# rogerbarton/optix-renderer

Measured on AMD Instinct MI355X. Metric: Msamples/sec (whole node) + traversal HBM GB/s, cbox 1024x1024 256spp, higher is better.
Workload: dtype f32; 1 GPU; Cornell box (diffuse-only) 1024x1024, 16400 spp, path_mis; config=c2, width=1024, height=1024, spp=16400, mode=wavefront, traversal=ordered, pools=2, gpu_max_hw_queues=8, parallelism=single GPU

## Files before the change

### include/nori_hip.h

```cpp
#ifndef NORI_HIP_H
#define NORI_HIP_H

#include <stddef.h>
#include <stdint.h>

#ifdef __cplusplus
extern "C" {
#endif

#define NH_OK 0
#define NH_ERR_INVALID 1
#define NH_ERR_IO 2
#define NH_ERR_DEVICE 3
#define NH_ERR_UNSUPPORTED 4
#define NH_ERR_STATE 5


enum { NH_SHAPE_MESH = 0, NH_SHAPE_SPHERE = 1 };
enum { NH_BSDF_DIFFUSE = 0, NH_BSDF_MIRROR = 1, NH_BSDF_DIELECTRIC = 2, NH_BSDF_MICROFACET = 3, NH_BSDF_DISNEY = 4 };
enum { NH_EMITTER_AREA = 0, NH_EMITTER_POINT = 1, NH_EMITTER_ENVMAP = 2, NH_EMITTER_SPOT = 3,
       NH_EMITTER_DIRECTIONAL = 4 };
enum { NH_INTEGRATOR_PATH_MIS = 0, NH_INTEGRATOR_PATH_MATS = 1, NH_INTEGRATOR_DIRECT_EMS = 2,
       NH_INTEGRATOR_DIRECT_MATS = 3, NH_INTEGRATOR_DIRECT_MIS = 4, NH_INTEGRATOR_DIRECT = 5,
       NH_INTEGRATOR_NORMALS = 6,
// ... 171 lines not shown
    float bbox_max[3];
} nh_bvh_node;

typedef struct nh_bvh_desc {
    uint32_t n_nodes;
    const nh_bvh_node *nodes;
    uint32_t n_indices;
    const uint32_t *indices;
    uint32_t n_shapes;
    const uint32_t *shape_offset;
    float bbox_min[3], bbox_max[3];
    uint32_t max_depth;
} nh_bvh_desc;


typedef struct nh_ray_soa {
    const float *ox, *oy, *oz;
    const float *dx, *dy, *dz;
    const float *mint, *maxt;
} nh_ray_soa;

typedef struct nh_hit_soa {
    uint8_t *hit;
    float *t, *u, *v;
    uint32_t *prim;
    uint32_t *shape;
} nh_hit_soa;


enum { NH_MODE_MEGAKERNEL = 0, NH_MODE_WAVEFRONT = 1 };
enum { NH_TRAVERSAL_REFERENCE = 0, NH_TRAVERSAL_ORDERED = 1, NH_TRAVERSAL_WIDE = 2 };

typedef struct nh_render_req {
    int32_t sample_begin;
    int32_t sample_end;
    uint64_t seed;
    int32_t n_blocks;
    const int32_t *blocks;
    int32_t mode;
    int32_t traversal;
    int32_t clear;
    int32_t collect_stats;
} nh_render_req;

#define NH_SMALL_TABLES_BYTES 4096

typedef struct nh_render_stats {
    double kernel_ms_path;
    double kernel_ms_splat;
    double kernel_ms_extend;
    double kernel_ms_shadow;
    double kernel_ms_shade;
    uint64_t launches_path, launches_splat, launches_extend, launches_shadow, launches_shade;
    uint64_t samples;
    uint64_t ray_queries;
    uint64_t nodes_visited;
    uint64_t boxes_tested;
    uint64_t prims_tested;
    uint64_t invalid_samples;
    uint64_t shadow_queries, shadow_nodes_visited, shadow_boxes_tested, shadow_prims_tested;
    uint64_t shade_state_bytes, extend_queue_bytes, shadow_queue_bytes, paths_shaded;
    double kernel_ms_tail;
    uint64_t launches_tail;
    uint64_t node_bytes;
    uint64_t tail_queries, tail_nodes_visited, tail_boxes_tested, tail_prims_tested;
    uint64_t tail_shadow_queries, tail_shadow_nodes_visited, tail_shadow_boxes_tested, tail_shadow_prims_tested;
    uint64_t lds_scene;
    uint64_t fused_bounce;
    uint64_t comm_inits;
    double kernel_ms_denoise;
    uint64_t launches_denoise;
    uint64_t tails_async;
    uint64_t pools_active;
    uint64_t trace_fused;
    uint64_t tail_cycles_body, tail_cycles_shadow, tail_cycles_closest, tail_cycles_head;
    uint64_t tail_bounces, tail_max_bounces;
    uint64_t tail_coop_cycles_body, tail_coop_cycles_shadow, tail_coop_cycles_closest, tail_coop_cycles_head;
    uint64_t tail_coop_bounces;
    uint64_t bounce_cycles_load, bounce_cycles_body, bounce_cycles_shadow, bounce_cycles_closest, bounce_cycles_head;
    uint64_t bounce_cycles_store, bounce_bounces;
    uint64_t bounce_traits;
    uint64_t primary_masks;
    uint64_t pair_kinds;
} nh_render_stats;

typedef struct nh_scene nh_scene;
typedef struct nh_bvh nh_bvh;
typedef struct nh_ctx nh_ctx;

int nh_scene_load_xml(const char *path, nh_scene **out);
int nh_scene_load_xml_index(const char *path, int32_t index, nh_scene **out);
int nh_scene_get_desc(const nh_scene *scene, nh_scene_desc *out);
int nh_scene_set_resolution(nh_scene *scene, int32_t width, int32_t height);
int nh_scene_set_sample_count(nh_scene *scene, int32_t spp);
int nh_scene_set_sampler(nh_scene *scene, int32_t type, int32_t initial_uniform);
int nh_scene_set_bsdf(nh_scene *scene, uint32_t shape, const nh_bsdf *bsdf);
uint32_t nh_scene_add_texture(nh_scene *scene, const nh_texture *tex, const float *texels);
int nh_scene_set_normal_map(nh_scene *scene, uint32_t shape, uint32_t texture);
int nh_scene_set_lens_draw_order(nh_scene *scene, int32_t order);
int nh_texture_decode(const uint8_t *rgba8, uint64_t n, int32_t srgb, float *out);
int nh_scene_set_integrator(nh_scene *scene, int32_t integrator);
typedef struct nh_photon_params {
    int32_t photon_count;
    float photon_radius;
} nh_photon_params;
int nh_scene_get_photon_params(const nh_scene *scene, nh_photon_params *out);
int nh_scene_set_photon_params(nh_scene *scene, const nh_photon_params *params);
typedef struct nh_av_params {
    float length;
} nh_av_params;
int nh_scene_get_av_params(const nh_scene *scene, nh_av_params *out);
int nh_scene_set_av_params(nh_scene *scene, const nh_av_params *params);
int nh_photon_tables(float *cos_theta, float *sin_theta, float *cos_phi, float *sin_phi, float *exp_table);
void nh_scene_free(nh_scene *scene);
const char *nh_host_last_error(void);
int nh_debug_transform(const char *request, float *out, int32_t cap);

int nh_bvh_build(const nh_scene_desc *scene, int32_t n_threads, nh_bvh **out);
int nh_bvh_get_desc(const nh_bvh *bvh, nh_bvh_desc *out);
void nh_bvh_free(nh_bvh *bvh);

int nh_primary_masks(const nh_camera *camera, const float *records, int32_t n_records, const int32_t *blocks,
                     int32_t n_blocks, uint64_t *masks, int32_t *built);
int32_t nh_primary_mask_pad(int32_t width, int32_t height);

int nh_pair_layout(const float *records, int32_t n_records, const int32_t *leaves, int32_t n_leaves, int32_t by_kind,
                   int32_t *slots, int32_t *leaf_pairs);

int nh_framebuffer_to_rgb(const float *rgbw, int32_t width, int32_t height, int32_t border, float *rgb);
int nh_write_pfm(const char *path, const float *rgb, int32_t width, int32_t height);
int nh_image_load_png(const char *path, uint8_t *rgba, size_t cap, int32_t *width, int32_t *height);
int nh_write_exr(const char *path, const float *rgb, int32_t width, int32_t height);
int nh_rgb_to_ldr(const float *rgb, int32_t width, int32_t height, uint8_t *rgb8);
int nh_write_png(const char *path, const float *rgb, int32_t width, int32_t height);

int nh_get_device_count(int *n);
int nh_create(int device, nh_ctx **out);
void nh_destroy(nh_ctx *ctx);
int nh_upload_scene(nh_ctx *ctx, const nh_scene_desc *scene);
int nh_upload_bvh(nh_ctx *ctx, const nh_bvh_desc *bvh);
int nh_trace_rays(nh_ctx *ctx, const nh_ray_soa *rays, int32_t n, int32_t any_hit, int32_t traversal, nh_hit_soa *out);
#define NH_ADAPTIVE_MAX_SAMPLES 133948
#define NH_ADAPTIVE_STAGING_BYTES ((size_t)4 << 30)
int nh_render(nh_ctx *ctx, const nh_render_req *req);
typedef struct nh_adaptive_stats {
    uint64_t total_samples;
    uint64_t passes;
    uint64_t max_passes;
    uint64_t n_blocks;
} nh_adaptive_stats;
int nh_get_adaptive_stats(nh_ctx *ctx, nh_adaptive_stats *out);
int nh_get_adaptive_variance(nh_ctx *ctx, float *out, size_t n_floats);
int nh_synchronize(nh_ctx *ctx);
int nh_get_framebuffer(nh_ctx *ctx, float *rgbw, size_t n_floats);
int nh_framebuffer_device_ptr(nh_ctx *ctx, void **dptr, size_t *n_floats);
int nh_get_stats(nh_ctx *ctx, nh_render_stats *out);
int nh_reset_stats(nh_ctx *ctx);
int nh_reduce_framebuffers(nh_ctx **ctxs, int32_t n, int32_t root);
int nh_denoise(nh_ctx *ctx, const nh_denoiser *params);
int nh_denoise_image(nh_ctx *ctx, float *rgbw, int32_t width, int32_t height, int32_t border,
                     const nh_denoiser *params);
enum { NH_BSDF_QUERY_EVAL = 0, NH_BSDF_QUERY_SAMPLE = 1 };
int nh_bsdf_query(nh_ctx *ctx, const nh_bsdf *bsdf, const float *albedo, int32_t mode, int32_t n, const float *wi,
                  const float *wo, const float *sample, float *wo_out, float *value, float *pdf, int32_t *measure);
enum { NH_EMITTER_QUERY_SAMPLE = 0, NH_EMITTER_QUERY_EVAL = 1, NH_EMITTER_QUERY_PDF = 2,
       NH_EMITTER_QUERY_SAMPLE_PHOTON = 3 };
#define NH_EMITTER_QUERY_SAMPLE_STRIDE 16
#define NH_EMITTER_QUERY_PHOTON_STRIDE 12
#define NH_EMITTER_QUERY_IN_STRIDE 9
int nh_emitter_query(nh_ctx *ctx, uint32_t emitter, int32_t mode, int32_t n, const float *ref, const float *sample,
                     float *out);
enum { NH_MEDIUM_QUERY_FREE_PATH = 0, NH_MEDIUM_QUERY_TRANSMITTANCE = 1, NH_MEDIUM_QUERY_PHASE_SAMPLE = 2,
       NH_MEDIUM_QUERY_PHASE_PDF = 3 };
int nh_medium_query(nh_ctx *ctx, uint32_t medium, int32_t mode, int32_t n, const float *in, float *out);


enum { NH_TEST_TTEST = 0, NH_TEST_CHI2TEST = 1 };
typedef struct nh_test_desc {
    int32_t type;
    float significance_level;
    int32_t sample_count;
    uint32_t n_angles;
    const float *angles;
    uint32_t n_references;
    const float *references;
    uint32_t n_scenes;
    uint32_t n_bsdfs;
    const nh_bsdf *bsdfs;
} nh_test_desc;
typedef struct nh_test nh_test;
int nh_test_load_xml(const char *path, nh_test **out);
int nh_test_get_desc(const nh_test *test, nh_test_desc *out);
void nh_test_free(nh_test *test);

int nh_students_t_test(double mean, double variance, double reference, int32_t n, double alpha, int32_t num_tests,
                       int32_t *accepted, double *p_value);

#define NH_RADIANCE_QUERY_MAX (1 << 24)
int nh_radiance_query(nh_ctx *ctx, uint64_t seed, int32_t n, const int32_t *pixel, const int32_t *sample,
                      const float *pixel_sample, float *rgb, float *jitter);
int nh_ttest_scene(nh_ctx *ctx, uint64_t seed, int64_t first, int32_t n, double *mean, double *variance,
                   float *luminance);
int nh_ttest_bsdf(nh_ctx *ctx, const nh_bsdf *bsdf, const float *albedo, float angle_deg, uint64_t first_draw,
                  int32_t n, double *mean, double *variance, float *luminance);
typedef struct nh_test_result {
    double mean, variance, reference, p_value;
    int32_t accepted;
    int32_t sample_count;
    float angle;
    int32_t pad;
// ... 31 lines not shown
```

### optix-renderer_amd/csrc/nh_ctx.h

```cpp
#pragma once
#include <hip/hip_runtime.h>
#include <rccl/rccl.h>

#include <algorithm>
#include <cstdint>
#include <deque>
#include <memory>
#include <string>
#include <vector>

#include "nh_internal.h"
#include "nori_hip.h"

constexpr int kRing = 4;
constexpr int kPools = 4;
constexpr int kTails = 3;
constexpr int kTailCap = 65536;
#ifndef NH_DEFAULT_POOLS
#define NH_DEFAULT_POOLS 2
#endif

struct WfJob {
    uint64_t seq;
    int s0, rounds;
// ... 66 lines not shown
    std::vector<int32_t> list_key;
    bool have_list = false;
    void release() {
        for (int *p : {pixel_list, pixel_map, block_ids, block_slot, color_slots}) (void)hipFree(p);
        *this = PixelList{};
    }
};

struct AdaptiveState {
    int n_blocks = 0, nbx = 0, nby = 0;
    int next_sample = -1;
    int4 *blocks = nullptr;
    int *block_rank = nullptr, *active_list = nullptr, *next = nullptr;
    AdBlock *state = nullptr;
    unsigned *counts = nullptr, *h_count = nullptr;
    int2 *pos = nullptr;
    float4 *rad = nullptr, *staging = nullptr;
    float2 *jit = nullptr;
    size_t slot_cap = 0;
    unsigned long long *stats = nullptr;
    std::vector<int4> h_blocks;
};

struct PhotonState {
    bool built = false;
    std::vector<void *> bufs;
    const float *tables = nullptr;
    std::vector<float> h_tables;
    float *pos = nullptr;
    uint2 *bytes = nullptr;
    uint32_t *path = nullptr;
    int *bounce = nullptr;
    nh_photon_stats stats{};
};

struct nh_ctx {
    uint64_t id = 0;
    std::shared_ptr<CommSet> comms;
    int device = 0;
    hipStream_t stream = nullptr;
    std::string err;
    std::vector<nh_shape> shapes;
    std::vector<float> V;
    std::vector<uint32_t> F;
    int width = 0, height = 0, border = 0, n_emitters = 0, integrator = 0;
    nh_filter filter{};
    nhd::DScene S{};
    nhd::DScene *d_scene = nullptr;
    nhd::Traversal tv{};
    std::vector<void *> scene_bufs, bvh_bufs;
    bool has_scene = false, has_bvh = false;
    int depth = 0;
    int depth_wide = 0;
    int wide_w = 4;
    int n_node_f4 = 0, n_leaves = 0, n_prim_f4 = 0;
    std::vector<uint32_t> bvh_indices, shape_offset;
    std::vector<int> shape_bsdf_type;
    std::vector<int> shape_bsdf_real;
    int n_bsdf_types = 0;
    bool disney = false;
    bool specular = false;
    bool textured = false;
    bool normal_mapped = false;
    bool diffuse_area = false;
    bool bsdfless = false, has_media = false;
    int sampler = 0, adaptive_initial_uniform = 0;
    AdaptiveState ad;
    PhotonState photon;
    bool av_set = false;
    AvLaunch av{};
    std::vector<void *> av_bufs;
    size_t av_cap = 0;
    int2 *av_spill = nullptr;
    int av_spill_depth = 0;
    std::vector<nhd::DShape> h_shapes;
    std::vector<nhd::DBsdf> h_bsdfs;
    std::vector<nhd::DEmitter> h_emitters;
    std::vector<float> h_area_cdf;
    int n_emit_faces = 0;
    float4 *small_image = nullptr;
    int small_tab[5] = {0, 0, 0, 0, 0};
    bool pair_kinds = false;
    float4 *small_image_ref = nullptr;
    nh_camera camera{};
    std::vector<float> h_prims;
    unsigned long long *pmask = nullptr;
    bool pmask_known = false;
    float *fb = nullptr;
    size_t fb_floats = 0;
    float *rec = nullptr;
    size_t rec_cap = 0;
    int *block_rank = nullptr;
    int nbx = 0, nby = 0;
    PixelList px;
    float4 *staging = nullptr;
    size_t staging_cap = 0;
    unsigned long long *counters = nullptr;
    nh_render_stats stats{};
    WfPool pools[kPools + kTails];
    std::deque<WfJob> jobs;
    uint64_t job_seq = 0, splat_seq = 0;
    hipEvent_t fb_ev = nullptr;
    bool fb_ev_set = false;
    uint64_t stats_comm_inits = 0;
};

inline void drop_primary_masks(nh_ctx *c) {
    (void)hipFree(c->pmask);
    c->pmask = nullptr;
    c->pmask_known = false;
}

#define NH_LAUNCH(c, fn) ((c)->disney ? nh_disney::nh::fn : nh::fn)

void pool_free(WfPool &p);
int pipeline_drain(nh_ctx *c);
int check_device(nh_ctx *c, const char *where);
int render_adaptive(nh_ctx *c, const nh_render_req *q);
void adaptive_release(nh_ctx *c);
void photon_release(nh_ctx *c, bool tables = false);
nhd::DDisney disney_record(const nh_bsdf &b);
void disney_set_record(nhd::DBsdf &o, const nhd::DDisney *rec);
int disney_upload(nh_ctx *c, std::vector<void *> &owner, const std::vector<nhd::DDisney> &recs,
                  const std::vector<float> &albedo, nhd::DDisney **out);

int query_bsdf_record(nh_ctx *c, std::vector<void *> &owner, const nh_bsdf *b, const float *albedo, nhd::DBsdf &o,
                      float alb[3]);

inline bool fail(nh_ctx *c, const std::string &m) {
    if (c) c->err = m;
    return false;
}

#define HIP_TRY(ctx, expr)                                                                               \
    do {                                                                                                 \
        hipError_t e_ = (expr);                                                                          \
        if (e_ != hipSuccess) {                                                                          \
            (ctx)->err = std::string(#expr) + ": " + hipGetErrorString(e_);                              \
            return NH_ERR_DEVICE;                                                                        \
        }                                                                                                \
    } while (0)

template <typename T>
int upload(nh_ctx *c, std::vector<void *> &owner, const T *src, size_t n, const T **dst) {
    void *p = nullptr;
    size_t bytes = (std::max<size_t>(n * sizeof(T), 16) + 15) / 16 * 16;
    HIP_TRY(c, hipMalloc(&p, bytes));
    owner.push_back(p);
    if (n) HIP_TRY(c, hipMemcpyAsync(p, src, n * sizeof(T), hipMemcpyHostToDevice, c->stream));
    *dst = reinterpret_cast<const T *>(p);
    return NH_OK;
}

inline void free_all(std::vector<void *> &v) {
    for (void *p : v) (void)hipFree(p);
    v.clear();
}
```

### optix-renderer_amd/csrc/nh_internal.h

```cpp
#pragma once
#include <hip/hip_runtime.h>
#include <stdint.h>

#include "nh_device.h"
#include "nh_traverse.h"
#include "nori_hip.h"

struct RayBatch {
    const float *ox, *oy, *oz, *dx, *dy, *dz, *mint, *maxt;
};
struct HitBatch {
    uint8_t *hit;
    float *t, *u, *v;
    int *k;
};
#ifndef NH_REC_STRIDE
#define NH_REC_STRIDE 3
#endif
constexpr int kRecFloats = NH_REC_STRIDE;

struct PathLaunch {
    int n_paths;
    int n_list;
    int s0;
// ... 67 lines not shown
constexpr int kStatTailCoopClk = 32;
constexpr int kStatBounceClk = 40;
__device__ __forceinline__ unsigned long long *stat_shard(unsigned long long *c) {
    return c + (blockIdx.x & (kStatShards - 1)) * kStatStride;
}
__device__ __forceinline__ void flush_stats(const nhd::TravStats &st, uint32_t queries, unsigned long long *counters) {
    unsigned long long v[4] = {queries, st.nodes, st.boxes, st.prims};
#pragma unroll
    for (int i = 0; i < 4; ++i) {
        unsigned long long x = v[i];
#pragma unroll
        for (int off = 32; off > 0; off >>= 1) x += __shfl_xor(x, off, 64);
        if ((threadIdx.x & 63) == 0) atomicAdd(&counters[i], x);
    }
}

namespace nh {
void launch_trace(const nhd::DScene *S, const nhd::Traversal &tv, const RayBatch &rb, const HitBatch &hb, int n,
                  bool any, bool ordered, bool stats, int depth, unsigned long long *ctr, hipStream_t st);
void launch_trace_wide(const nhd::DScene *S, const nhd::Traversal &tv, const RayBatch &rb, const HitBatch &hb, int n,
                       bool any, bool ordered, bool stats, int2 *spill, int spill_depth, unsigned long long *ctr,
                       hipStream_t st, int wide = 4);
void launch_path(const nhd::DScene *S, const nhd::Traversal &tv, const PathLaunch &L, bool ordered, bool stats,
                 int depth, bool pm, hipStream_t st);
void launch_splat(const SplatLaunch &P, hipStream_t st);
void launch_av_primary(const nhd::DScene *S, const AvLaunch &L, hipStream_t st);
void launch_av_shade(const nhd::DScene *S, const nhd::Traversal &tv, const AvLaunch &L, hipStream_t st);
void launch_av_resolve(const AvLaunch &L, int bound, hipStream_t st);
bool splat_uses_staging(int border, int reach);
void launch_count_invalid(const float *rec, size_t n, unsigned long long *out, hipStream_t st);
void launch_denoise_variance(const DenoiseLaunch &P, hipStream_t st);
int denoise_band_rows();
int denoise_max_chunk();
int tree_top_nodes();
size_t denoise_tile_static_lds();
void launch_denoise_band(const DenoiseLaunch &P, int L, int n_bands, size_t tile_bytes, hipStream_t st);
void launch_denoise_copy(const float4 *src, int src_stride, float4 *dst, int dst_stride, int width, int height,
                         hipStream_t st);
}

constexpr int kQueueShards = 8, kCountStride = 32;

struct WfBuf {
    float4 *ray_o;
    float4 *ray_d;
    float4 *hit;
    uint64_t *rng;
    float4 *li;
    float4 *thr;
    float4 *pend;
    uint8_t *occl;
};
struct WfState {
    WfBuf buf[2];
    float4 *sh_o, *sh_d;
    int *sh_slot;
    unsigned *counts;
};
constexpr int kCountGroup = kQueueShards * kCountStride;
constexpr int kCountSlot = 4 * kCountGroup;

struct WfLaunch {
    WfState st;
    int n_paths, n_list, s0;
    uint64_t seed;
    const int *pixel_list;
    float *rec;
    float2 *jit;
    int in_q;
    int first;
    int cam_rays;
    unsigned *cnt_in;
    unsigned *cnt_out;
    int seg_cap;
    int small_nodes, small_leaves, small_prims;
    int small_frames;
    const float4 *small_image;
    int small_tab[5];
    uint32_t *trav_spill;
    int spill_depth;
    unsigned long long *counters;
    const unsigned long long *pmask;
    int pmask_nbx;
};
constexpr int kPersistentBlocks = 256 * 16;
constexpr size_t kSmallSceneBytes = 16384;
constexpr int kSmallFramesMaxPrims = 256;
constexpr size_t kSmallTablesBytes = NH_SMALL_TABLES_BYTES;
namespace nh {
void launch_wf_trace(const nhd::DScene *S, const nhd::Traversal &tv, const WfLaunch &L, bool ordered, bool stats,
                     bool shadow, bool persistent, int wide, int bound, int depth, hipStream_t st);
void launch_wf_trace2(const nhd::DScene *S, const nhd::Traversal &tv, const WfLaunch &L, bool ordered, bool stats,
                      int wide, int bound, hipStream_t st);
void launch_wf_camera_rays(const nhd::DScene *S, const WfLaunch &L, int bound, hipStream_t st);
void launch_wf_shade(const nhd::DScene *S, const nhd::Traversal &tv, const WfLaunch &L, bool sort, bool nmap, int bound,
                     hipStream_t st);
void launch_wf_bounce(const nhd::DScene *S, const nhd::Traversal &tv, const WfLaunch &L, bool ordered, bool stats,
                      bool sort, int bound, hipStream_t st);
void launch_wf_bounce_rr(const nhd::DScene *S, const nhd::Traversal &tv, const WfLaunch &L, bool ordered, bool stats, bool sort,
                         bool lean, bool nmap, bool trait, int bound, hipStream_t st);
void launch_wf_tail_rr(const nhd::DScene *S, const nhd::Traversal &tv, const WfLaunch &L, bool ordered, bool stats, int bound,
                       bool specular, bool lean, bool nmap, bool trait, hipStream_t st);
void launch_wf_bounce_trait(const nhd::DScene *S, const nhd::Traversal &tv, const WfLaunch &L, bool stats, int bound,
                            hipStream_t st);
void launch_wf_tail_trait(const nhd::DScene *S, const nhd::Traversal &tv, const WfLaunch &L, bool stats, int bound,
                          int coop, hipStream_t st);
void launch_wf_tail(const nhd::DScene *S, const nhd::Traversal &tv, const WfLaunch &L, bool ordered, bool stats,
                    int wide, int bound, int depth, hipStream_t st);
void launch_wf_pack_rr(const WfLaunch &L, const WfBuf &dst, unsigned *dst_counts, int bound, hipStream_t st);
void launch_small_image(const nhd::Traversal &tv, int n_prim_f4, const int2 *slots, int pairs_off, int frames_off,
                        float4 *image, hipStream_t st);
void launch_wf_counts(const unsigned *src, unsigned *host_dst, int n_copy, unsigned *zero, int n_zero, hipStream_t st);
}

namespace nh_disney {
namespace nh {
void launch_path(const nhd::DScene *S, const nhd::Traversal &tv, const PathLaunch &L, bool ordered, bool stats,
                 int depth, bool pm, hipStream_t st);
void launch_wf_shade(const nhd::DScene *S, const nhd::Traversal &tv, const WfLaunch &L, bool sort, bool nmap, int bound,
                     hipStream_t st);
void launch_wf_bounce(const nhd::DScene *S, const nhd::Traversal &tv, const WfLaunch &L, bool ordered, bool stats,
                      bool sort, int bound, hipStream_t st);
void launch_wf_bounce_rr(const nhd::DScene *S, const nhd::Traversal &tv, const WfLaunch &L, bool ordered, bool stats, bool sort,
                         bool lean, bool nmap, bool trait, int bound, hipStream_t st);
void launch_wf_tail_rr(const nhd::DScene *S, const nhd::Traversal &tv, const WfLaunch &L, bool ordered, bool stats, int bound,
                       bool specular, bool lean, bool nmap, bool trait, hipStream_t st);
void launch_wf_tail(const nhd::DScene *S, const nhd::Traversal &tv, const WfLaunch &L, bool ordered, bool stats,
                    int wide, int bound, int depth, hipStream_t st);
void launch_disney_fold(nhd::DDisney *recs, const float *albedo, int n, hipStream_t st);
struct BsdfQuery {
    nhd::DBsdf bsdf;
    float albedo[3];
    int mode, n;
    const float *wi, *wo, *sample;
    float *wo_out, *value, *pdf;
    int *measure;
};
void launch_bsdf_query(const BsdfQuery &q, hipStream_t st);
struct EmitterQuery {
    int emitter, mode, n;
    const float *ref, *in;
    float *out;
};
void launch_emitter_query(const nhd::DScene *S, const EmitterQuery &q, hipStream_t st);
void launch_vol_path(const nhd::DScene *S, const nhd::Traversal &tv, const PathLaunch &L, bool mis, bool stats, int depth,
                     hipStream_t st);
struct MediumQuery {
    int medium, mode, n;
    const float *in;
    float *out;
};
void launch_medium_query(const nhd::DScene *S, const MediumQuery &q, hipStream_t st);
}
}

struct PhotonTrace {
    uint64_t seed, k0;
    int n_paths;
    long long *counts;
    const long long *offsets;
    long long base;
    int cap;
    float *pos;
    uint2 *bytes;
    uint32_t *path;
    int *bounce;
// ... 110 lines not shown
```

### optix-renderer_amd/csrc/nh_layout.h

```cpp
#pragma once

namespace nhd {

constexpr int kLensLo = 256, kLensHi = 65536;

constexpr int kPrimSphere = 1, kPrimLeafEnd = 2, kPrimMatShift = 2;
constexpr int kPrimIsolated = 16;

constexpr int kWideF4 = 8;
constexpr int kWideEmpty = (int)0x80000000;

constexpr int kMaxStack = 128;

}
```

### optix-renderer_amd/csrc/nh_pipeline.hip

```cpp
#include <cmath>
#include <cstdlib>
#include <cstring>
#include <thread>
#include <type_traits>

#include "../host/gpu_layout.h"
#include "nh_ctx.h"


constexpr size_t kWfBytesPerPath = 2 * (16 * 6 + 8 + 1) + 36;

static int pool_alloc(nh_ctx *c, WfPool &p, size_t n, size_t rec_n, size_t staging_f4, bool jit = false) {
    if (!p.stream) {
        if (!p.h_counts && hipHostMalloc(reinterpret_cast<void **>(&p.h_counts),
                                         (kRing * 2 * kCountGroup + kCountSlot) * sizeof(unsigned)) != hipSuccess) {
            p.h_counts = nullptr;
            return fail(c, "hipHostMalloc failed"), NH_ERR_DEVICE;
        }
        for (hipEvent_t &e : p.copy_ev)
            if (!e) HIP_TRY(c, hipEventCreateWithFlags(&e, hipEventDisableTiming));
        for (hipEvent_t *e : {&p.ev_begin, &p.ev_path, &p.ev_splat0, &p.ev_splat})
            if (!*e) HIP_TRY(c, hipEventCreate(e));
        if (!p.ev_handoff) HIP_TRY(c, hipEventCreateWithFlags(&p.ev_handoff, hipEventDisableTiming));
        HIP_TRY(c, hipStreamCreateWithFlags(&p.stream, hipStreamNonBlocking));
// ... 112 lines not shown
}

static int pool_start(nh_ctx *c, WfPool &p, const WfJob &job) {
    WfJob j = job;
    j.staged = splat_staged(c);
    const char *jv = std::getenv("NH_SPLAT_JITTER");
    j.jit = jv && std::strcmp(jv, "stored") == 0;
    const int n_paths = j.rounds * c->px.n_list;
    const size_t staging_f4 = (size_t)j.rounds * c->px.n_blocks * block_px(c, j.staged);
    int rc = pool_alloc(c, p, (size_t)n_paths, (size_t)n_paths, staging_f4, j.jit);
    if (rc) return rc;
    for (int i = 0; i < active_pools(c); ++i) {
        WfPool &o = c->pools[i];
        if (&o == &p || o.state != WfPool::IDLE) continue;
        if ((rc = pool_alloc(c, o, (size_t)n_paths, (size_t)n_paths, staging_f4, j.jit))) return rc;
    }
    if (active_pools(c) > 1 && tail_async_enabled())
        for (int i = kPools; i < kPools + kTails; ++i) {
            WfPool &o = c->pools[i];
            if (o.state != WfPool::IDLE) continue;
            if ((rc = pool_alloc(c, o, (size_t)kTailCap, (size_t)n_paths, staging_f4, j.jit))) return rc;
        }
    p.job = j;
    WfLaunch &L = p.L;
    L = WfLaunch{};
    L.st = p.wf;
    L.n_paths = n_paths;
    L.n_list = c->px.n_list;
    L.s0 = j.s0;
    L.seed = j.seed;
    L.pixel_list = c->px.pixel_list;
    L.rec = p.rec;
    L.jit = j.jit ? p.jit : nullptr;
    L.counters = c->counters;
    const size_t scene_bytes = 16 * (size_t)(c->n_node_f4 + c->n_prim_f4) + 8 * (size_t)c->n_leaves;
    bool small = scene_bytes <= kSmallSceneBytes;
    if (const char *e = std::getenv("NH_LDS_SCENE")) small = small && e[0] != '0';
    if (small) {
        L.small_nodes = c->n_node_f4;
        L.small_leaves = c->n_leaves;
        L.small_prims = c->n_prim_f4;
        L.small_frames = c->n_prim_f4 / 3 <= kSmallFramesMaxPrims;
        if (const char *e = std::getenv("NH_LDS_FRAMES")) L.small_frames = L.small_frames && e[0] != '0';
        L.small_image = j.stats && c->small_image_ref ? c->small_image_ref : c->small_image;
        for (int i = 0; i < 5; ++i) L.small_tab[i] = c->small_tab[i];
    }
    const int per_chunk = 256;
    const int max_chunks = (n_paths + per_chunk - 1) / per_chunk;
    L.seg_cap = (max_chunks + kQueueShards - 1) / kQueueShards * per_chunk;
    p.persistent = c->depth > 20;
    if (const char *e = std::getenv("NH_PERSISTENT")) p.persistent = e[0] == '1';
    p.wide = p.persistent && j.ordered && c->tv.wnodes != nullptr;
    if (const char *e = std::getenv("NH_WIDE")) p.wide = p.wide && e[0] != '0';
    if (p.wide && !j.ordered) return fail(c, "wavefront pool: the wide traversal needs an ordered job"), NH_ERR_STATE;
    p.trace2 = p.wide && scene_bytes <= (size_t)256 << 20;
    if (const char *e = std::getenv("NH_TRACE2")) p.trace2 = p.wide && e[0] != '0';
    c->stats.trace_fused = p.trace2 ? 1 : 0;
    const int spill_words = p.wide ? 2 * c->depth_wide : (c->depth + 1) / 2 * 2;
    if (p.persistent && p.spill_words < spill_words) {
        HIP_TRY(c, hipStreamSynchronize(p.stream));
        (void)hipFree(p.spill);
        p.spill = nullptr;
        p.spill_words = 0;
        HIP_TRY(c, hipMalloc(&p.spill, (size_t)kPersistentBlocks * 128 * spill_words * sizeof(uint32_t)));
        p.spill_words = spill_words;
    }
    p.fused = small && !p.persistent && c->depth <= 16;
    if (const char *e = std::getenv("NH_FUSED")) p.fused = p.fused && e[0] != '0';
    p.sorted = p.fused && c->n_bsdf_types > 1;
    p.rr = p.fused;
    if (const char *e = std::getenv("NH_RR_AHEAD")) p.rr = p.fused && e[0] != '0';
    p.shade_sorted = false;
    if (const char *e = std::getenv("NH_SORT_SHADE")) p.shade_sorted = !p.fused && e[0] == '1';
    if (const char *e = std::getenv("NH_SORT")) p.sorted = p.fused && e[0] == '1';
    p.trait = p.rr && c->diffuse_area && c->small_tab[0] > 0 && j.ordered && !p.sorted;
    if (const char *e = std::getenv("NH_BOUNCE_TRAITS")) p.trait = p.trait && e[0] != '0';
    c->stats.bounce_traits = p.rr ? (p.trait ? 2 : 1) : 0;
    const char *pm = std::getenv("NH_PRIMARY_MASKS");
    const bool masks = p.rr && c->pmask && !j.stats && !(pm && pm[0] == '0');
    L.pmask = masks ? c->pmask : nullptr;
    L.pmask_nbx = c->nbx;
    c->stats.primary_masks = masks ? 1 : 0;
    c->stats.pair_kinds = p.fused && c->pair_kinds && !j.stats ? 1 : 0;
    c->stats.fused_bounce = p.fused ? 1 : 0;
    c->stats.node_bytes = p.wide ? 16 * nhd::kWideF4 * (c->wide_w / 4) : 64;
    c->stats.lds_scene = small && !p.persistent && c->depth <= 16 ? 1 : 0;
    L.trav_spill = p.spill;
    L.spill_depth = p.spill_words;
    p.tail_at = p.fused ? std::min<int64_t>(std::max<int64_t>(n_paths / 1024, 8192), 16384)
                        : std::min<int64_t>(std::max<int64_t>(n_paths / 64, 8192), 262144);
    if (const char *e = std::getenv("NH_TAIL")) p.tail_at = std::atoll(e);
    p.drain_at = std::max<int64_t>(n_paths / 8, p.tail_at);
    HIP_TRY(c, hipEventRecord(p.ev_begin, p.stream));
    unsigned *h_init = p.h_counts + kRing * 2 * kCountGroup;
    std::memset(h_init, 0, kCountSlot * sizeof(unsigned));
    h_init[0] = (unsigned)n_paths;
    HIP_TRY(c, hipMemcpyAsync(p.wf.counts, h_init, kCountSlot * sizeof(unsigned), hipMemcpyHostToDevice, p.stream));
    p.in_e.assign(1, (uint64_t)n_paths);
    p.in_s.assign(1, 0);
    p.it = 0;
    p.tail = false;
    p.draining = false;
    p.state = WfPool::ENQUEUE;
    return NH_OK;
}

static void chunk_swap(WfPool &a, WfPool &b) {
    std::swap(a.h_counts, b.h_counts);
    std::swap(a.copy_ev, b.copy_ev);
    std::swap(a.events, b.events);
    std::swap(a.ev_begin, b.ev_begin);
    std::swap(a.ev_path, b.ev_path);
    std::swap(a.ev_splat0, b.ev_splat0);
    std::swap(a.ev_splat, b.ev_splat);
    std::swap(a.job, b.job);
    std::swap(a.L, b.L);
    std::swap(a.persistent, b.persistent);
    std::swap(a.wide, b.wide);
    std::swap(a.trace2, b.trace2);
    std::swap(a.tail, b.tail);
    std::swap(a.draining, b.draining);
    std::swap(a.fused, b.fused);
    std::swap(a.sorted, b.sorted);
    std::swap(a.rr, b.rr);
    std::swap(a.trait, b.trait);
    std::swap(a.shade_sorted, b.shade_sorted);
    std::swap(a.tail_at, b.tail_at);
    std::swap(a.drain_at, b.drain_at);
    std::swap(a.it, b.it);
    std::swap(a.in_e, b.in_e);
    std::swap(a.in_s, b.in_s);
    std::swap(a.rec, b.rec);
    std::swap(a.rec_cap, b.rec_cap);
    std::swap(a.jit, b.jit);
    std::swap(a.jit_cap, b.jit_cap);
    std::swap(a.staging, b.staging);
    std::swap(a.staging_cap, b.staging_cap);
}

static WfPool *free_tail_slot(nh_ctx *c, const WfPool &p, int bound) {
    if (!p.rr || bound > kTailCap || active_pools(c) < 2) return nullptr;
    if (!tail_async_enabled()) return nullptr;
    for (int i = kPools; i < kPools + kTails; ++i)
        if (c->pools[i].state == WfPool::IDLE) return &c->pools[i];
    return nullptr;
}

static int pool_handoff(nh_ctx *c, WfPool &p, WfPool &T, int bound, hipEvent_t *ev) {
    int rc = pool_alloc(c, T, (size_t)kTailCap, 0, 0);
    if (rc) return rc;
    HIP_TRY(c, hipMemsetAsync(T.wf.counts, 0, kCountSlot * sizeof(unsigned), p.stream));
    nh::launch_wf_pack_rr(p.L, T.wf.buf[0], T.wf.counts, bound, p.stream);
    HIP_TRY(c, hipGetLastError());
    HIP_TRY(c, hipEventRecord(p.ev_handoff, p.stream));
    chunk_swap(p, T);
    WfLaunch &L = T.L;
    L.st = T.wf;
    L.in_q = 0;
    L.cnt_in = T.wf.counts;
    HIP_TRY(c, hipStreamWaitEvent(T.stream, p.ev_handoff, 0));
    HIP_TRY(c, hipEventRecord(ev[1], T.stream));
    HIP_TRY(c, hipEventRecord(ev[2], T.stream));
    NH_LAUNCH(c, launch_wf_tail_rr)(c->d_scene, c->tv, L, T.job.ordered, T.job.stats, bound, c->specular,
                          !c->specular && !c->textured, c->normal_mapped, T.trait, T.stream);
    HIP_TRY(c, hipGetLastError());
    HIP_TRY(c, hipEventRecord(ev[3], T.stream));
// ... 433 lines not shown
    c->av_cap = paths;
    c->av_spill_depth = spill_depth;
    return NH_OK;
}

static int av_chunk(nh_ctx *c, const nh_render_req *q, const PathLaunch &P) {
    AvLaunch L = c->av;
    L.n_paths = P.n_paths;
    L.n_list = P.n_list;
    L.s0 = P.s0;
    L.seed = P.seed;
    L.pixel_list = P.pixel_list;
    L.rec = P.rec;
    const bool wide = av_wide(c, q), ordered = q->traversal != NH_TRAVERSAL_REFERENCE, stats = q->collect_stats != 0;
    const auto batch = [&](float *const r[8], const HitBatch &hb, int n, bool any) {
        const RayBatch rb{r[0], r[1], r[2], r[3], r[4], r[5], r[6], r[7]};
        unsigned long long *ctr = c->counters + (any ? kStatAny : 0);
        if (wide) nh::launch_trace_wide(c->d_scene, c->tv, rb, hb, n, any, true, stats, c->av_spill, c->av_spill_depth, ctr,
                                        c->stream, c->wide_w);
        else nh::launch_trace(c->d_scene, c->tv, rb, hb, n, any, ordered, stats, c->depth, ctr, c->stream);
    };
    HIP_TRY(c, hipMemsetAsync(L.q_count, 0, sizeof(unsigned), c->stream));
    nh::launch_av_primary(c->d_scene, L, c->stream);
    batch(L.ray, L.hit, L.n_paths, false);
    nh::launch_av_shade(c->d_scene, c->tv, L, c->stream);
    HIP_TRY(c, hipGetLastError());
    int n_queue = L.n_paths;
    if (stats) {
        unsigned n = 0;
        HIP_TRY(c, hipMemcpyAsync(&n, L.q_count, sizeof(n), hipMemcpyDeviceToHost, c->stream));
        HIP_TRY(c, hipStreamSynchronize(c->stream));
        n_queue = (int)n;
    }
    HitBatch occl{};
    occl.hit = L.q_hit;
    batch(L.q_ray, occl, n_queue, true);
    nh::launch_av_resolve(L, n_queue, c->stream);
    return NH_OK;
}

extern "C" {

int nh_render(nh_ctx *c, const nh_render_req *q) {
    if (!c || !q) return NH_ERR_INVALID;
    if (!c->has_scene || !c->has_bvh) return fail(c, "nh_render: scene and BVH must be uploaded"), NH_ERR_STATE;
    if (q->sample_end < q->sample_begin || q->sample_begin < 0) return fail(c, "invalid sample range"), NH_ERR_INVALID;
    if (c->S.dof && q->sample_end > nhd::kLensLo * nhd::kLensHi)
        return fail(c, "depth of field: sample rounds beyond 2^24"), NH_ERR_UNSUPPORTED;
    if ((c->integrator == NH_INTEGRATOR_PATH_MIS || c->integrator == NH_INTEGRATOR_DIRECT_MIS) && c->n_emitters == 0)
        return fail(c, "No Emitter in scene!"), NH_ERR_INVALID;
    if (q->mode != NH_MODE_MEGAKERNEL && q->mode != NH_MODE_WAVEFRONT) return fail(c, "unknown render mode"), NH_ERR_INVALID;
    const bool volumetric = c->integrator == NH_INTEGRATOR_PATH_VOL_MATS || c->integrator == NH_INTEGRATOR_PATH_VOL_MIS;
    if (!volumetric && (c->bsdfless || c->has_media))
        return fail(c, "the scene has a participating medium or a shape without a BSDF: only the path_vol_mats and "
                       "path_vol_mis integrators render it"), NH_ERR_UNSUPPORTED;
    if (c->integrator == NH_INTEGRATOR_PATH_VOL_MIS && c->n_emitters == 0)
        return fail(c, "No Emitter in scene!"), NH_ERR_INVALID;
    const bool photon = c->integrator == NH_INTEGRATOR_PHOTONMAPPER;
    if (photon && !c->photon.built)
        return fail(c, "nh_render: the photon mapper needs a photon map (nh_photon_map_build)"), NH_ERR_STATE;
    if (photon && c->sampler == NH_SAMPLER_ADAPTIVE)
        return fail(c, "photonmapper: the adaptive sampler is not supported"), NH_ERR_UNSUPPORTED;
    if (c->integrator == NH_INTEGRATOR_AV && !c->av_set)
        return fail(c, "nh_render: the av integrator needs its length (nh_set_av_params)"), NH_ERR_STATE;
    if (c->integrator == NH_INTEGRATOR_ENVMAPTESTER && c->S.envmap < 0)
        return fail(c, "This integrator requires an env map."), NH_ERR_INVALID;
    const bool av_split = q->mode == NH_MODE_WAVEFRONT && c->integrator == NH_INTEGRATOR_AV;
    const bool wavefront = q->mode == NH_MODE_WAVEFRONT && c->integrator <= NH_INTEGRATOR_PATH_MATS;
    if (q->traversal < NH_TRAVERSAL_REFERENCE || q->traversal > NH_TRAVERSAL_WIDE)
        return fail(c, "unknown traversal"), NH_ERR_INVALID;
    if (c->border > 4) return fail(c, "reconstruction filters wider than border 4 are not supported"), NH_ERR_UNSUPPORTED;
    HIP_TRY(c, hipSetDevice(c->device));
    int rc = NH_OK;
    if (!wavefront || q->collect_stats || q->clear || c->sampler == NH_SAMPLER_ADAPTIVE) rc = pipeline_drain(c);
    if (rc) return rc;
    if (c->sampler == NH_SAMPLER_ADAPTIVE) return render_adaptive(c, q);
    rc = ensure_pixel_list(c, q);
    if (rc) return rc;
    if (wavefront && (rc = ensure_primary_masks(c))) return rc;
    c->stats.node_bytes = 64;
    if (av_split && av_wide(c, q)) c->stats.node_bytes = 16 * nhd::kWideF4 * (c->wide_w / 4);
    c->stats.primary_masks = 0;
    c->stats.pair_kinds = 0;
    c->stats.trace_fused = 0;
    c->stats.lds_scene = 0;
    c->stats.fused_bounce = 0;
    if (q->clear) {
        HIP_TRY(c, hipMemsetAsync(c->fb, 0, c->fb_floats * sizeof(float), c->stream));
        HIP_TRY(c, hipEventRecord(c->fb_ev, c->stream));
        c->fb_ev_set = true;
    }
    const int rounds = q->sample_end - q->sample_begin;
    if (rounds == 0 || c->px.n_list == 0) return NH_OK;
    if (q->collect_stats)
        HIP_TRY(c, hipMemsetAsync(c->counters, 0, kStatShards * kStatStride * sizeof(unsigned long long), c->stream));
    const size_t per_round = (size_t)c->px.n_list;
    const char *jv = std::getenv("NH_SPLAT_JITTER");
    const size_t rec_bytes = kRecFloats * 4 + (wavefront && jv && std::strcmp(jv, "stored") == 0 ? 8 : 0);
    const size_t per_round_bytes = per_round * rec_bytes + (size_t)c->px.n_blocks * block_px(c, splat_staged(c)) * 16 +
                                   (wavefront ? per_round * kWfBytesPerPath : 0) +
                                   (av_split ? per_round * av_bytes_per_path(c, q) : 0);
    size_t budget = wavefront ? (size_t)24 << 30 : (size_t)1 << 30;
    if (const char *e = std::getenv(wavefront ? "NH_WF_BUDGET_MB" : "NH_RECORD_BUDGET_MB"))
        budget = (size_t)std::max(1L, std::atol(e)) << 20;
    if (wavefront) {
        size_t free_b = 0, total_b = 0;
        if (hipMemGetInfo(&free_b, &total_b) == hipSuccess) {
            size_t held = 0;
            for (const WfPool &p : c->pools)
                held += p.cap * kWfBytesPerPath + p.rec_cap * kRecFloats * 4 + p.jit_cap * 8 + p.staging_cap * sizeof(float4);
            const int shares = active_pools(c) + (active_pools(c) > 1 && tail_async_enabled() ? kTails : 0);
            const size_t avail = (size_t)((double)(free_b + held) * 0.85) / (size_t)shares;
            budget = std::min(budget, std::max(avail, per_round_bytes));
        }
    }
    int chunk = (int)std::max<size_t>(1, std::min<size_t>((size_t)rounds, budget / per_round_bytes));
    while ((size_t)chunk * per_round > (size_t)0x7fffffff) chunk = std::max(1, chunk / 2);
    if (wavefront) {
        if (per_round > ((size_t)1 << 26))
            return fail(c, "wavefront mode renders at most 2^26 pixels per context"), NH_ERR_UNSUPPORTED;
        chunk = std::min(chunk, (int)(((size_t)1 << 26) / per_round));
    }

    if (wavefront) {
        HIP_TRY(c, hipStreamSynchronize(c->stream));
        for (int s = q->sample_begin; s < q->sample_end; s += chunk)
            c->jobs.push_back(WfJob{c->job_seq++, s, std::min(chunk, q->sample_end - s), q->seed,
                                    q->traversal != NH_TRAVERSAL_REFERENCE, q->collect_stats != 0});
        rc = q->collect_stats ? pipeline_drain(c) : pipeline_run(c, false);
        if (rc) return rc;
        if (int e = check_device(c, "nh_render")) return e;
    } else {
        if (c->rec_cap < (size_t)chunk * per_round) {
            (void)hipFree(c->rec);
            c->rec = nullptr;
            c->rec_cap = 0;
            const size_t cap = (size_t)chunk * per_round;
            HIP_TRY(c, hipMalloc(&c->rec, cap * kRecFloats * sizeof(float)));
            c->rec_cap = cap;
        }
        if (av_split && (rc = av_reserve(c, (size_t)chunk * per_round, av_wide(c, q)))) return rc;
        const bool staged = splat_staged(c);
        if (c->staging_cap < (size_t)chunk * c->px.n_blocks * block_px(c, staged)) {
            (void)hipFree(c->staging);
            c->staging = nullptr;
            c->staging_cap = 0;
            const size_t cap = (size_t)chunk * c->px.n_blocks * block_px(c, staged);
            HIP_TRY(c, hipMalloc(&c->staging, cap * sizeof(float4)));
            c->staging_cap = cap;
        }
        struct Ev {
            hipEvent_t a, b, d;
        };
        std::vector<Ev> evs;
        for (int s = q->sample_begin; s < q->sample_end; s += chunk) {
            const int k = std::min(chunk, q->sample_end - s);
            PathLaunch L{};
            L.n_paths = k * c->px.n_list;
            L.n_list = c->px.n_list;
            L.s0 = s;
            L.seed = q->seed;
            L.pixel_list = c->px.pixel_list;
            L.rec = c->rec;
            L.counters = c->counters;
            Ev ev;
            HIP_TRY(c, hipEventCreate(&ev.a));
// ... 86 lines not shown
```

### optix-renderer_amd/csrc/nh_traverse.h

```cpp
#pragma once
#include "nh_device.h"

namespace nhd {

struct Hit {
    float t, u, v;
    int k;
};

struct TravStats {
    uint32_t nodes, boxes, prims;
};

NHD bool box_test(float mnx, float mny, float mnz, float mxx, float mxy, float mxz, F3 o, F3 d, F3 r, float mint,
                  float maxt, float &near_out) {
    float near_t = -INFINITY, far_t = INFINITY;
    if (d.x == 0) {
        if (o.x < mnx || o.x > mxx) return false;
    } else {
        float t1 = (mnx - o.x) * r.x, t2 = (mxx - o.x) * r.x;
        if (t1 > t2) { float tmp = t1; t1 = t2; t2 = tmp; }
        near_t = e_max(t1, near_t);
        far_t = e_min(t2, far_t);
        if (!(near_t <= far_t)) return false;
    }
    if (d.y == 0) {
        if (o.y < mny || o.y > mxy) return false;
    } else {
        float t1 = (mny - o.y) * r.y, t2 = (mxy - o.y) * r.y;
        if (t1 > t2) { float tmp = t1; t1 = t2; t2 = tmp; }
        near_t = e_max(t1, near_t);
        far_t = e_min(t2, far_t);
        if (!(near_t <= far_t)) return false;
    }
    if (d.z == 0) {
        if (o.z < mnz || o.z > mxz) return false;
    } else {
        float t1 = (mnz - o.z) * r.z, t2 = (mxz - o.z) * r.z;
        if (t1 > t2) { float tmp = t1; t1 = t2; t2 = tmp; }
        near_t = e_max(t1, near_t);
        far_t = e_min(t2, far_t);
        if (!(near_t <= far_t)) return false;
    }
    near_out = near_t;
    return mint <= far_t && near_t <= maxt;
}

NHD float rcp_rn(float x) {
    const float r = __builtin_amdgcn_rcpf(x);
    const float e = __builtin_fmaf(-x, r, 1.0f);
    return __builtin_fmaf(e, r, r);
}
NHD float tri_inv_det(float det) {
    float r = rcp_rn(det);
    if (__builtin_expect(fabsf(det) >= 0x1p126f, 0)) r = 1.0f / det;
    return r;
}
NHD float dir_rcp(float x) {
    const float a = fabsf(x);
    if (__builtin_expect(a >= 0x1p-125f && a < 0x1p126f, 1)) return rcp_rn(x);
    return 1.0f / x;
}

NHD bool tri_test(float4 a, float4 b, float4 c, F3 o, F3 d, float mint, float maxt, float &t, float &u, float &v) {
    const F3 p0 = f3(a.x, a.y, a.z), e1 = sub(f3(b.x, b.y, b.z), p0), e2 = sub(f3(c.x, c.y, c.z), p0);
    F3 pvec = cross(d, e2);
    float det = dot(e1, pvec);
    if (det > -1e-8f && det < 1e-8f) return false;
    float inv_det = tri_inv_det(det);
    F3 tvec = sub(o, p0);
    u = dot(tvec, pvec) * inv_det;
    if (u < 0.0f || u > 1.0f) return false;
    F3 qvec = cross(tvec, e1);
    v = dot(d, qvec) * inv_det;
    if (v < 0.0f || u + v > 1.0f) return false;
    t = dot(e2, qvec) * inv_det;
    return t >= mint && t <= maxt;
}

typedef float f2 __attribute__((ext_vector_type(2)));
struct P3 {
    f2 x, y, z;
};
NHD P3 psub(P3 a, P3 b) { return P3{a.x - b.x, a.y - b.y, a.z - b.z}; }
// ... 49 lines not shown
    const float ax = (mnx - o.x) * r.x, bx = (mxx - o.x) * r.x;
    const float ay = (mny - o.y) * r.y, by = (mxy - o.y) * r.y;
    const float az = (mnz - o.z) * r.z, bz = (mxz - o.z) * r.z;
    const float near_t = fmaxf(fmaxf(fminf(ax, bx), fminf(ay, by)), fminf(az, bz));
    const float far_t = fminf(fminf(fmaxf(ax, bx), fmaxf(ay, by)), fmaxf(az, bz));
    near_out = near_t;
    return (near_t <= far_t) & (mint <= far_t) & (near_t <= maxt);
}

NHD void box_test_finite_pair(f2 mnx, f2 mny, f2 mnz, f2 mxx, f2 mxy, f2 mxz, float o_x, float o_y, float o_z,
                              float r_x, float r_y, float r_z, float mint, float maxt, bool &hit0, bool &hit1,
                              float &near0, float &near1) {
    const f2 ox{o_x, o_x}, oy{o_y, o_y}, oz{o_z, o_z}, rx{r_x, r_x}, ry{r_y, r_y}, rz{r_z, r_z};
    const f2 ax = (mnx - ox) * rx, bx = (mxx - ox) * rx;
    const f2 ay = (mny - oy) * ry, by = (mxy - oy) * ry;
    const f2 az = (mnz - oz) * rz, bz = (mxz - oz) * rz;
    const float n0 = fmaxf(fmaxf(fminf(ax.x, bx.x), fminf(ay.x, by.x)), fminf(az.x, bz.x));
    const float f0 = fminf(fminf(fmaxf(ax.x, bx.x), fmaxf(ay.x, by.x)), fmaxf(az.x, bz.x));
    const float n1 = fmaxf(fmaxf(fminf(ax.y, bx.y), fminf(ay.y, by.y)), fminf(az.y, bz.y));
    const float f1 = fminf(fminf(fmaxf(ax.y, bx.y), fmaxf(ay.y, by.y)), fmaxf(az.y, bz.y));
    near0 = n0;
    near1 = n1;
    hit0 = (n0 <= f0) & (mint <= f0) & (n0 <= maxt);
    hit1 = (n1 <= f1) & (mint <= f1) & (n1 <= maxt);
}

NHD bool sphere_test(float4 a, F3 o, F3 d, float mint, float maxt, float &t) {
    F3 L = sub(o, f3(a.x, a.y, a.z));
    float qa = dot(d, d);
    float qb = 2.f * dot(d, L);
    float qc = dot(L, L) - a.w * a.w;
    float discr = qb * qb - 4.f * qa * qc;
    if (discr < 0.f) return false;
    const float tmin = (-qb - f_sqrt(discr)) / 2 / qa;
    const float tmax = (-qb + f_sqrt(discr)) / 2 / qa;
    if (mint <= tmin && maxt >= tmin) { t = tmin; return true; }
    if (mint <= tmax && maxt >= tmax) { t = tmax; return true; }
    return false;
}

NHD void sphere_test_pair(f2 cx, f2 cy, f2 cz, f2 rad, F3 o, F3 d, f2 &tmin, f2 &tmax, bool &ok0, bool &ok1) {
    const P3 po{f2{o.x, o.x}, f2{o.y, o.y}, f2{o.z, o.z}}, pd{f2{d.x, d.x}, f2{d.y, d.y}, f2{d.z, d.z}};
    const P3 L = psub(po, P3{cx, cy, cz});
    const float qa = dot(d, d);
    const f2 qb = 2.f * pdot(pd, L);
    const f2 qc = pdot(L, L) - rad * rad;
    const f2 discr = qb * qb - (4.f * qa) * qc;
    ok0 = !(discr.x < 0.f);
    ok1 = !(discr.y < 0.f);
    tmin = tmax = f2{0.f, 0.f};
    if (ok0 | ok1) {
        const f2 s{f_sqrt(discr.x), f_sqrt(discr.y)};
        const f2 lo = (-qb - s) / 2, hi = (-qb + s) / 2;
        tmin = f2{lo.x / qa, lo.y / qa};
        tmax = f2{hi.x / qa, hi.y / qa};
    }
}
NHD bool sphere_in_range(float tmin, float tmax, float mint, float maxt, float &t) {
    const bool near_ok = mint <= tmin && maxt >= tmin;
    t = near_ok ? tmin : tmax;
    return near_ok || (mint <= tmax && maxt >= tmax);
}

NHD void accept_hit(bool hit, float t, float u, float v, int k, float &maxt, Hit &best, bool &found) {
    const bool up = hit && (t < maxt || k > best.k);
    maxt = up ? t : maxt;
    best.t = up ? t : best.t;
    best.u = up ? u : best.u;
    best.v = up ? v : best.v;
    best.k = up ? k : best.k;
    found = found || up;
}

struct Traversal {
    const float4 *nodes;
    const int2 *leaves;
    const float4 *prims;
    const float4 *wnodes;
    const float4 *ppairs;
    const int2 *pleaves;
    const float4 *frames;
    int n_top;
};
constexpr int kPairF4 = 6;

NHD bool prim_is_tri(float4 c) { return (__float_as_int(c.w) & kPrimSphere) == 0; }
NHD int prim_material(float4 c) { return (__float_as_int(c.w) >> kPrimMatShift) & 3; }

template <bool ANY, bool STATS, bool PAIRS = false, bool MASKED = false>
NHD bool leaf_test(const Traversal &tv, int leaf, F3 o, F3 d, float mint, float &maxt, Hit &best, bool &found,
                   TravStats &st, unsigned long long cand = ~0ull) {
    if constexpr (PAIRS && !STATS) {
        const int2 pl = tv.pleaves[leaf];
        if (pl.y) {
            const float4 *pp = tv.ppairs + (size_t)kPairF4 * pl.x;
            for (int i = 0, n = pl.y & 0xffff; i < n; ++i, pp += kPairF4) {
                const float4 q5 = pp[5];
                const int k0 = __float_as_int(q5.z), k1 = __float_as_int(q5.w);
                if constexpr (MASKED)
                    if (!(((cand >> (k0 & 63)) | (cand >> (k1 & 63))) & 1ull)) continue;
                const float4 q0 = pp[0], q1 = pp[1], q2 = pp[2], q3 = pp[3], q4 = pp[4];
                const P3 p0{f2{q0.x, q0.y}, f2{q0.z, q0.w}, f2{q1.x, q1.y}};
                const P3 e1{f2{q2.x, q2.y}, f2{q2.z, q2.w}, f2{q3.x, q3.y}};
                const P3 e2{f2{q3.z, q3.w}, f2{q4.x, q4.y}, f2{q4.z, q4.w}};
                f2 pt, pu, pv;
                bool ok0, ok1;
                tri_test_pair_e(p0, e1, e2, o, d, mint, pt, pu, pv, ok0, ok1);
                if (ANY) {
                    if ((ok0 && pt.x <= maxt) || (ok1 && pt.y <= maxt)) return true;
                    continue;
                }
                accept_hit(ok0 && pt.x <= maxt, pt.x, pu.x, pv.x, k0, maxt, best, found);
                accept_hit(ok1 && pt.y <= maxt, pt.y, pu.y, pv.y, k1, maxt, best, found);
            }
            for (int i = 0, n = pl.y >> 16; i < n; ++i, pp += kPairF4) {
                const float4 q5 = pp[5];
                const int k0 = __float_as_int(q5.z), k1 = __float_as_int(q5.w);
                if constexpr (MASKED)
                    if (!(((cand >> (k0 & 63)) | (cand >> (k1 & 63))) & 1ull)) continue;
                const float4 q0 = pp[0], q1 = pp[1];
                f2 tmin, tmax;
                bool ok0, ok1;
                sphere_test_pair(f2{q0.x, q0.y}, f2{q0.z, q0.w}, f2{q1.x, q1.y}, f2{q1.z, q1.w}, o, d, tmin, tmax, ok0, ok1);
                if (!(ok0 | ok1)) continue;
                float t0, t1;
                if (ANY) {
                    if ((sphere_in_range(tmin.x, tmax.x, mint, maxt, t0) && ok0) ||
                        (sphere_in_range(tmin.y, tmax.y, mint, maxt, t1) && ok1))
                        return true;
                    continue;
                }
                const bool h0 = sphere_in_range(tmin.x, tmax.x, mint, maxt, t0) && ok0;
                accept_hit(h0, t0, 0.f, 0.f, k0, maxt, best, found);
                const bool h1 = sphere_in_range(tmin.y, tmax.y, mint, maxt, t1) && ok1;
                accept_hit(h1, t1, 0.f, 0.f, k1, maxt, best, found);
            }
            return false;
        }
    }
    const int2 lf = tv.leaves[leaf];
    if constexpr (PAIRS) {
        for (int k = lf.x, e = lf.x + lf.y; k < e; k += 2) {
            if constexpr (MASKED && !STATS)
                if (!((cand >> (k & 63)) & 3ull)) continue;
            const float4 *pp = tv.ppairs + (size_t)kPairF4 * k;
            const float4 q0 = pp[0], q1 = pp[1], q2 = pp[2], q3 = pp[3], q4 = pp[4], q5 = pp[5];
            const P3 p0{f2{q0.x, q0.y}, f2{q0.z, q0.w}, f2{q1.x, q1.y}};
            const P3 e1{f2{q2.x, q2.y}, f2{q2.z, q2.w}, f2{q3.x, q3.y}};
            const P3 e2{f2{q3.z, q3.w}, f2{q4.x, q4.y}, f2{q4.z, q4.w}};
            f2 pt, pu, pv;
            bool ok0, ok1;
            tri_test_pair_e(p0, e1, e2, o, d, mint, pt, pu, pv, ok0, ok1);
            const bool has1 = k + 1 < e;
            if (!STATS && !((__float_as_int(q5.x) | (has1 ? __float_as_int(q5.y) : 0)) & kPrimSphere)) {
                if (ANY) {
                    if ((ok0 && pt.x <= maxt) || (has1 && ok1 && pt.y <= maxt)) return true;
                    continue;
                }
                const bool h0 = ok0 && pt.x <= maxt;
                const bool u0 = h0 && (pt.x < maxt || k > best.k);
                maxt = u0 ? pt.x : maxt;
                best.t = u0 ? pt.x : best.t;
                best.u = u0 ? pu.x : best.u;
                best.v = u0 ? pv.x : best.v;
                best.k = u0 ? k : best.k;
                const bool h1 = has1 && ok1 && pt.y <= maxt;
                const bool u1 = h1 && (pt.y < maxt || k + 1 > best.k);
// ... 141 lines not shown
    if (fin) {
        box_test_finite_pair(f2{l0, r0}, f2{l1, r1}, f2{l2, r2}, f2{l3, r3}, f2{l4, r4}, f2{l5, r5}, o.x, o.y, o.z, r.x,
                             r.y, r.z, mint, maxt, hl, hr, nl, nr);
    } else {
        hl = box_test(l0, l1, l2, l3, l4, l5, o, d, r, mint, maxt, nl);
        hr = box_test(r0, r1, r2, r3, r4, r5, o, d, r, mint, maxt, nr);
    }
}

template <int DEPTH, bool ORDERED, bool ANY, bool STATS, bool PAIRS = false, int G = 1, bool RCP = false,
          bool MASKED = false>
NHD bool trace(const Traversal &tv, const DScene &S, F3 o, F3 d, float mint, float maxt, Hit &best, uint32_t *stk,
               int stride, TravStats &st, unsigned long long cand = ~0ull) {
    if (mint == kEps) mint = e_max(mint, mint * e_max(fabsf(o.x), e_max(fabsf(o.y), fabsf(o.z))));
    const bool lead = G == 1 || (threadIdx.x & (G - 1)) == 0;
    best.k = -1;
    best.t = INFINITY;
    if (S.root_kind == 0 || maxt < mint) return false;
    const F3 r = RCP ? f3(dir_rcp(d.x), dir_rcp(d.y), dir_rcp(d.z)) : f3(1.0f / d.x, 1.0f / d.y, 1.0f / d.z);
    const bool fin = isfinite(r.x) & isfinite(r.y) & isfinite(r.z);
    bool found = false;
    float near_t;
    if (STATS && lead) st.boxes++;
    if (fin ? !box_test_finite(S.root_min[0], S.root_min[1], S.root_min[2], S.root_max[0], S.root_max[1],
                               S.root_max[2], o, r, mint, maxt, near_t)
            : !box_test(S.root_min[0], S.root_min[1], S.root_min[2], S.root_max[0], S.root_max[1], S.root_max[2], o,
                        d, r, mint, maxt, near_t))
        return false;
    if (S.root_kind == 2) {
        bool any = leaf_any<ANY, STATS, PAIRS, G, MASKED>(tv, 0, o, d, mint, maxt, best, found, st, cand);
        return ANY ? any : found;
    }
    int sp = 0;
    int cur = 0;
    for (;;) {
        while (cur >= 0) {
            const float *nf = node_f(tv, cur);
            const int ref_l = node_ref(nf, 0), ref_r = node_ref(nf, 1);
            if (STATS && lead) { st.nodes++; st.boxes += 2; }
            float nl, nr;
            bool hl, hr;
            node_box_tests(nf, o, d, r, mint, maxt, fin, hl, hr, nl, nr);
            int next;
            if (hl && hr) {
                const bool right_first = ORDERED && nr < nl;
                stk[sp * stride] = ((uint32_t)cur << 1) | (right_first ? 0u : 1u);
                ++sp;
                next = right_first ? ref_r : ref_l;
            } else if (hl) {
                next = ref_l;
            } else if (hr) {
                next = ref_r;
            } else {
                break;
            }
            if (next >= 0) {
                cur = next;
                continue;
            }
            if (leaf_any<ANY, STATS, PAIRS, G, MASKED>(tv, ~next, o, d, mint, maxt, best, found, st, cand)) return true;
            break;
        }
        cur = -1;
        while (sp > 0) {
            --sp;
            const uint32_t e = stk[sp * stride];
            const int parent = (int)(e >> 1), side = (int)(e & 1u);
            const float *nf = node_f(tv, parent);
            if (STATS && lead) st.boxes++;
            if (!child_box_test(nf, side, o, d, r, mint, maxt, near_t, fin)) continue;
            const int ref = node_ref(nf, side);
            if (ref >= 0) {
                cur = ref;
                break;
            }
            if (leaf_any<ANY, STATS, PAIRS, G, MASKED>(tv, ~ref, o, d, mint, maxt, best, found, st, cand)) return true;
        }
        if (cur < 0) break;
    }
    (void)DEPTH;
    return ANY ? false : found;
}

template <bool STATS, int G = 1>
NHD bool iso_sphere_hit(const Traversal &tv, int k_prev, F3 o, F3 d, float mint, float maxt, Hit &best,
                        TravStats &st) {
    if (k_prev < 0) return false;
    const float4 c = tv.prims[3 * k_prev + 2];
    if (!(__float_as_int(c.w) & kPrimIsolated)) return false;
    if (mint == kEps) mint = e_max(mint, mint * e_max(fabsf(o.x), e_max(fabsf(o.y), fabsf(o.z))));
    if (maxt < mint) return false;
    const float4 a = tv.prims[3 * k_prev];
    const float lim = a.w + tv.prims[3 * k_prev + 1].x;
    if (!(fabsf(o.x - a.x) <= lim && fabsf(o.y - a.y) <= lim && fabsf(o.z - a.z) <= lim)) return false;
    float t;
    if (!sphere_test(a, o, d, mint, maxt, t) || !(t >= 2.f * mint)) return false;
    best.t = t;
    best.u = 0.f;
    best.v = 0.f;
    best.k = k_prev;
    if (STATS && (G == 1 || (threadIdx.x & (G - 1)) == 0)) st.prims++;
    return true;
}

template <int DEPTH, bool ORDERED, bool STATS, bool PAIRS = false, int G = 1, bool ISO = true, bool RCP = false>
NHD bool trace_next(const Traversal &tv, const DScene &S, int k_prev, F3 o, F3 d, float mint, float maxt, Hit &best,
                    uint32_t *stk, int stride, TravStats &st) {
#ifndef NH_AB_NO_ISO
    if (ISO && S.iso_spheres && S.root_kind != 0 && iso_sphere_hit<STATS, G>(tv, k_prev, o, d, mint, maxt, best, st))
        return true;
#endif
    return trace<DEPTH, ORDERED, false, STATS, PAIRS, G, RCP>(tv, S, o, d, mint, maxt, best, stk, stride, st);
}



template <int K>
struct RingStack {
    static_assert((K & (K - 1)) == 0, "K must be a power of two");
    uint32_t *lds;
    int stride;
    uint32_t *glob;
    NHD void push(int i, uint32_t e) {
        uint32_t *slot = lds + (i & (K - 1)) * stride;
        if (i >= K) glob[i - K] = *slot;
        *slot = e;
    }
    NHD uint32_t pop(int i) {
        uint32_t *slot = lds + (i & (K - 1)) * stride;
        const uint32_t e = *slot;
        if (i >= K) *slot = glob[i - K];
        return e;
    }
};

template <bool ORDERED, bool ANY, bool STATS, class Stack>
struct Tracer {
    F3 o, d, r;
    float mint, maxt;
    int cur;
    int k, kend;
    int sp;
    bool found, done;
    bool fin;
    Hit best;

    NHD void begin(const DScene &S, const Traversal &tv, F3 o_, F3 d_, float mint_, float maxt_, TravStats &st) {
        o = o_;
        d = d_;
        mint = mint_;
        maxt = maxt_;
        if (mint == kEps) mint = e_max(mint, mint * e_max(fabsf(o.x), e_max(fabsf(o.y), fabsf(o.z))));
        best.k = -1;
        best.t = INFINITY;
        found = false;
        done = true;
        sp = 0;
        cur = -1;
        k = kend = 0;
        if (S.root_kind == 0 || maxt < mint) return;
        r = f3(1.0f / d.x, 1.0f / d.y, 1.0f / d.z);
        fin = isfinite(r.x) & isfinite(r.y) & isfinite(r.z);
        float near_t;
        if (STATS) st.boxes++;
        if (fin ? !box_test_finite(S.root_min[0], S.root_min[1], S.root_min[2], S.root_max[0], S.root_max[1],
                                   S.root_max[2], o, r, mint, maxt, near_t)
                : !box_test(S.root_min[0], S.root_min[1], S.root_min[2], S.root_max[0], S.root_max[1], S.root_max[2],
                            o, d, r, mint, maxt, near_t))
            return;
        done = false;
        if (S.root_kind == 2) {
            const int2 lf = tv.leaves[0];
            k = lf.x;
            kend = lf.x + lf.y;
        } else {
            cur = 0;
        }
    }

    NHD void step(const Traversal &tv, Stack &stk, TravStats &st) {
        if (k < kend) {
            const float4 a = tv.prims[3 * k], b = tv.prims[3 * k + 1], c = tv.prims[3 * k + 2];
            if (STATS) st.prims++;
            float t, u = 0.f, v = 0.f;
            const bool hit = prim_is_tri(c) ? tri_test(a, b, c, o, d, mint, maxt, t, u, v)
                                                        : sphere_test(a, o, d, mint, maxt, t);
            if (hit) {
                if (ANY) {
                    found = true;
                    done = true;
                    return;
                }
                if (t < maxt || k > best.k) {
                    found = true;
                    maxt = t;
// ... 486 lines not shown
```

### optix-renderer_amd/csrc/nh_upload.hip

```cpp
#include <cmath>
#include <cstdlib>
#include <cstring>

#include "../host/gpu_layout.h"
#include "nh_ctx.h"

using nhd::DBsdf;
using nhd::DEmitter;
using nhd::DShape;

static_assert(sizeof(nh::f4) == sizeof(float4) && alignof(float4) % alignof(nh::f4) == 0, "nh::f4 is float4's layout");
static_assert(sizeof(nh::i2) == sizeof(int2) && alignof(int2) % alignof(nh::i2) == 0, "nh::i2 is int2's layout");
static_assert(sizeof(nh::u64x2) == sizeof(ulonglong2) && alignof(ulonglong2) % alignof(nh::u64x2) == 0,
              "nh::u64x2 is ulonglong2's layout");
static_assert((int)nhd::BSDF_DIELECTRIC == (int)NH_BSDF_DIELECTRIC, "the isolated-sphere marking reads NH_BSDF_*");

nhd::DDisney disney_record(const nh_bsdf &b) {
    nhd::DDisney o;
    std::memset(&o, 0, sizeof(o));
    o.metallic = b.metallic; o.subsurface = b.subsurface; o.specular = b.specular; o.roughness = b.roughness;
    o.specular_tint = b.specular_tint; o.anisotropic = b.anisotropic; o.sheen = b.sheen; o.sheen_tint = b.sheen_tint;
    o.clearcoat = b.clearcoat; o.clearcoat_gloss = b.clearcoat_gloss;
    return o;
}
// ... 280 lines not shown
    for (int i = 0; i < 3; ++i) S.ndir[i] = d->normals_direction[i];
    std::memcpy(S.s2c, d->camera.sample_to_camera, sizeof(S.s2c));
    std::memcpy(S.c2w, d->camera.camera_to_world, sizeof(S.c2w));
    {
        float ow[4];
        const float z = 0.0f;
        for (int i = 0; i < 4; ++i) {
            float acc = S.c2w[4 * i] * z;
            acc = acc + S.c2w[4 * i + 1] * z;
            acc = acc + S.c2w[4 * i + 2] * z;
            acc = acc + S.c2w[4 * i + 3] * 1.0f;
            ow[i] = acc;
        }
        for (int i = 0; i < 3; ++i) S.cam_o[i] = ow[i] / ow[3];
    }
    S.inv_w = d->camera.inv_output_size[0];
    S.inv_h = d->camera.inv_output_size[1];
    S.near_clip = d->camera.near_clip;
    S.far_clip = d->camera.far_clip;
    S.width = d->camera.width;
    S.height = d->camera.height;
    S.dof = d->camera.lens_radius > 1e-4f ? 1 : 0;
    S.lens_radius = d->camera.lens_radius;
    S.focal_distance = d->camera.focal_distance;
    S.lens_rtl = d->camera.lens_draw_order == NH_LENS_DRAWS_RTL ? 1 : 0;
    S.lens_pix = S.lens_lo = nullptr;
    S.lens_hi = nullptr;
    if (S.dof) {
        const nh::LensTables lt = nh::lens_tables(S.width, S.height);
        const nh::u64x2 *pix = nullptr, *lo = nullptr;
        if ((rc = upload(c, c->scene_bufs, lt.pix.data(), lt.pix.size(), &pix))) return rc;
        if ((rc = upload(c, c->scene_bufs, lt.lo.data(), lt.lo.size(), &lo))) return rc;
        if ((rc = upload(c, c->scene_bufs, lt.hi.data(), lt.hi.size(), &S.lens_hi))) return rc;
        S.lens_pix = reinterpret_cast<const ulonglong2 *>(pix);
        S.lens_lo = reinterpret_cast<const ulonglong2 *>(lo);
        HIP_TRY(c, hipStreamSynchronize(c->stream));
    }
    S.filter_radius = d->filter.radius;
    S.lookup = d->filter.lookup_factor;
    S.border = d->filter.border;
    std::memcpy(S.table, d->filter.table, sizeof(S.table));

    c->shapes.assign(d->shapes, d->shapes + d->n_shapes);
    c->shape_bsdf_type.clear();
    c->shape_bsdf_real.clear();
    unsigned types = 0;
    for (uint32_t i = 0; i < d->n_shapes; ++i) {
        const int t = d->shapes[i].bsdf < 0 ? NH_BSDF_DIFFUSE : d->bsdfs[d->shapes[i].bsdf].type;
        c->shape_bsdf_real.push_back(t);
        types |= 1u << t;
    }
    int disney_key = 0;
    for (int k : {NH_BSDF_MICROFACET, NH_BSDF_MIRROR, NH_BSDF_DIELECTRIC, NH_BSDF_DIFFUSE})
        if (!(types & (1u << k))) {
            disney_key = k;
            break;
        }
    for (int t : c->shape_bsdf_real) c->shape_bsdf_type.push_back(t == NH_BSDF_DISNEY ? disney_key : t);
    c->disney = (types & (1u << NH_BSDF_DISNEY)) != 0;
    c->disney = c->disney || !dx.empty();
    c->n_bsdf_types = __builtin_popcount(types);
    c->specular = (types & ((1u << NH_BSDF_MIRROR) | (1u << NH_BSDF_DIELECTRIC))) != 0;
    c->textured = false;
    for (uint32_t i = 0; i < d->n_bsdfs; ++i) c->textured = c->textured || d->bsdfs[i].albedo_texture != 0;
    c->normal_mapped = false;
    for (uint32_t i = 0; i < d->n_shapes; ++i) c->normal_mapped = c->normal_mapped || d->shapes[i].normal_map != 0;
    c->textured = c->textured || c->normal_mapped;
    c->diffuse_area = S.integrator == NH_INTEGRATOR_PATH_MIS && !c->textured && !S.dof && d->envmap < 0 &&
                      d->n_emitters > 0;
    for (uint32_t i = 0; i < d->n_bsdfs; ++i) c->diffuse_area = c->diffuse_area && d->bsdfs[i].type == NH_BSDF_DIFFUSE;
    for (uint32_t i = 0; i < d->n_emitters; ++i) {
        const nh_emitter &e = d->emitters[i];
        c->diffuse_area = c->diffuse_area && e.type == NH_EMITTER_AREA && e.shape >= 0 &&
                          (uint32_t)e.shape < d->n_shapes && ds[e.shape].ef_off >= 0;
    }
    for (uint32_t i = 0; i < d->n_shapes; ++i)
        c->diffuse_area = c->diffuse_area && d->shapes[i].emitter < (int32_t)d->n_emitters;
    c->h_shapes = ds;
    c->h_bsdfs = db;
    c->h_emitters = de;
    c->h_area_cdf.assign(d->area_cdf, d->area_cdf + d->n_area_cdf);
    c->n_emit_faces = (int)ef_tri.size();
    c->small_image = c->small_image_ref = nullptr;
    c->pair_kinds = false;
    c->V.assign(d->V, d->V + 3 * nv);
    c->F.assign(d->F, d->F + 3 * (size_t)d->n_faces);
    c->width = d->camera.width;
    c->height = d->camera.height;
    c->border = d->filter.border;
    c->filter = d->filter;
    c->n_emitters = (int)d->n_emitters;
    c->integrator = S.integrator;
    if (d->sampler != NH_SAMPLER_INDEPENDENT && d->sampler != NH_SAMPLER_ADAPTIVE)
        return fail(c, "unknown sampler"), NH_ERR_INVALID;
    c->sampler = d->sampler;
    c->adaptive_initial_uniform = std::max(1, (int)d->adaptive_initial_uniform);
    adaptive_release(c);
    photon_release(c);
    c->av_set = false;

    (void)hipFree(c->fb);
    c->fb = nullptr;
    c->fb_floats = 4 * (size_t)(c->width + 2 * c->border) * (size_t)(c->height + 2 * c->border);
    HIP_TRY(c, hipMalloc(&c->fb, c->fb_floats * sizeof(float)));
    HIP_TRY(c, hipMemsetAsync(c->fb, 0, c->fb_floats * sizeof(float), c->stream));
    auto rank = nh::spiral_rank(c->width, c->height, 32, c->nbx, c->nby);
    (void)hipFree(c->block_rank);
    HIP_TRY(c, hipMalloc(&c->block_rank, rank.size() * sizeof(int)));
    HIP_TRY(c, hipMemcpyAsync(c->block_rank, rank.data(), rank.size() * sizeof(int), hipMemcpyHostToDevice, c->stream));
    HIP_TRY(c, hipStreamSynchronize(c->stream));
    c->has_scene = true;
    return NH_OK;
}

static int build_small_image(nh_ctx *c, const nh::GpuBvh &g) {
    c->small_image = c->small_image_ref = nullptr;
    c->pair_kinds = false;
    for (int &v : c->small_tab) v = 0;
    const size_t scene_bytes = 16 * (size_t)(c->n_node_f4 + c->n_prim_f4) + 8 * (size_t)c->n_leaves;
    if (scene_bytes > kSmallSceneBytes) return NH_OK;
    const int n = c->n_prim_f4 / 3;
    const int leaves_f4 = (c->n_leaves + 1) / 2;
    const int pairs_off = c->n_node_f4 + c->n_prim_f4 + leaves_f4;
    const bool frames = n <= kSmallFramesMaxPrims;
    std::vector<float4> tab;
    if (c->diffuse_area) {
        std::vector<nhd::DShape> sh = c->h_shapes;
        std::vector<float> cdf;
        for (const nhd::DEmitter &e : c->h_emitters) {
            nhd::DShape &s = sh[e.shape];
            if ((size_t)s.pdf_off + s.n_faces + 1 > c->h_area_cdf.size()) return fail(c, "area CDF out of range"), NH_ERR_INVALID;
            const int off = (int)cdf.size();
            cdf.insert(cdf.end(), c->h_area_cdf.begin() + s.pdf_off, c->h_area_cdf.begin() + s.pdf_off + s.n_faces + 1);
            s.pdf_off = off;
        }
        cdf.resize((cdf.size() + 3) / 4 * 4, 0.f);
        const size_t bytes = sh.size() * sizeof(nhd::DShape) + c->h_bsdfs.size() * sizeof(nhd::DBsdf) +
                             c->h_emitters.size() * sizeof(nhd::DEmitter) + cdf.size() * sizeof(float) +
                             3 * (size_t)c->n_emit_faces * sizeof(float4);
        if (bytes <= kSmallTablesBytes) {
            static_assert(sizeof(nhd::DShape) % 16 == 0 && sizeof(nhd::DBsdf) % 16 == 0 && sizeof(nhd::DEmitter) % 16 == 0,
                          "table records are whole float4s");
            c->small_tab[0] = (int)(sh.size() * sizeof(nhd::DShape) / 16);
            c->small_tab[1] = (int)(c->h_bsdfs.size() * sizeof(nhd::DBsdf) / 16);
            c->small_tab[2] = (int)(c->h_emitters.size() * sizeof(nhd::DEmitter) / 16);
            c->small_tab[3] = (int)(cdf.size() / 4);
            c->small_tab[4] = 3 * c->n_emit_faces;
            tab.resize((size_t)c->small_tab[0] + c->small_tab[1] + c->small_tab[2] + c->small_tab[3]);
            char *w = reinterpret_cast<char *>(tab.data());
            std::memcpy(w, sh.data(), sh.size() * sizeof(nhd::DShape));
            w += sh.size() * sizeof(nhd::DShape);
            std::memcpy(w, c->h_bsdfs.data(), c->h_bsdfs.size() * sizeof(nhd::DBsdf));
            w += c->h_bsdfs.size() * sizeof(nhd::DBsdf);
            std::memcpy(w, c->h_emitters.data(), c->h_emitters.size() * sizeof(nhd::DEmitter));
            w += c->h_emitters.size() * sizeof(nhd::DEmitter);
            std::memcpy(w, cdf.data(), cdf.size() * sizeof(float));
        }
    }
    const int tab_f4 = (int)tab.size() + c->small_tab[4];
    const int pleaves_off = pairs_off + nhd::kPairF4 * n, tab_off = pleaves_off + leaves_f4;
    const int frames_off = tab_off + tab_f4;
    const size_t total = (size_t)frames_off + (frames ? 3 * (size_t)n : 0);
    const auto d2d = [&](float4 *dst, const void *src, size_t bytes) {
        return bytes ? hipMemcpyAsync(dst, src, bytes, hipMemcpyDeviceToDevice, c->stream) : hipSuccess;
    };
    const char *pk = std::getenv("NH_PAIR_KINDS");
    c->pair_kinds = n > 0 && !(pk && pk[0] == '0');
    for (int pass = 0; pass < (c->pair_kinds ? 2 : 1); ++pass) {
        const bool by_kind = c->pair_kinds && pass == 0;
        const nh::PairLayout pl = nh::pair_layout(g.leaves.data(), c->n_leaves, g.prims.data(), n, by_kind);
        float4 *img = nullptr;
        HIP_TRY(c, hipMalloc(&img, std::max<size_t>(total, 1) * sizeof(float4)));
        c->bvh_bufs.push_back(img);
        HIP_TRY(c, hipMemsetAsync(img, 0, std::max<size_t>(total, 1) * sizeof(float4), c->stream));
        HIP_TRY(c, d2d(img, c->tv.nodes, 16 * (size_t)c->n_node_f4));
        HIP_TRY(c, d2d(img + c->n_node_f4, c->tv.prims, 16 * (size_t)c->n_prim_f4));
        HIP_TRY(c, d2d(img + c->n_node_f4 + c->n_prim_f4, c->tv.leaves, 8 * (size_t)c->n_leaves));
        if (n > 0) {
            const nh::i2 *slots = nullptr;
            if (int rc = upload(c, c->bvh_bufs, pl.slots.data(), pl.slots.size(), &slots)) return rc;
            nh::launch_small_image(c->tv, c->n_prim_f4, reinterpret_cast<const int2 *>(slots), pairs_off,
                                   frames ? frames_off : -1, img, c->stream);
            HIP_TRY(c, hipGetLastError());
        }
        if (c->n_leaves > 0)
            HIP_TRY(c, hipMemcpyAsync(img + pleaves_off, pl.leaves.data(), 8 * (size_t)c->n_leaves, hipMemcpyHostToDevice,
                                      c->stream));
        if (!tab.empty()) {
            float4 *t = img + tab_off;
            HIP_TRY(c, hipMemcpyAsync(t, tab.data(), tab.size() * sizeof(float4), hipMemcpyHostToDevice, c->stream));
            HIP_TRY(c, d2d(t + tab.size(), c->S.emit_faces, 16 * (size_t)c->small_tab[4]));
        }
        HIP_TRY(c, hipStreamSynchronize(c->stream));
        (pass == 0 ? c->small_image : c->small_image_ref) = img;
    }
    return NH_OK;
}

int nh_set_av_params(nh_ctx *c, const nh_av_params *params) {
    if (!c) return NH_ERR_INVALID;
    if (!params || std::isnan(params->length)) return fail(c, "nh_set_av_params: invalid av parameters"), NH_ERR_INVALID;
    if (!c->has_scene) return fail(c, "nh_set_av_params: no scene uploaded"), NH_ERR_STATE;
    HIP_TRY(c, hipSetDevice(c->device));
    if (int rc = pipeline_drain(c)) return rc;
    HIP_TRY(c, hipStreamSynchronize(c->stream));
    c->S.av_length = params->length;
    if (c->d_scene && c->has_bvh)
        HIP_TRY(c, hipMemcpy(reinterpret_cast<char *>(c->d_scene) + offsetof(nhd::DScene, av_length), &c->S.av_length,
                             sizeof(float), hipMemcpyHostToDevice));
    c->av_set = true;
    return NH_OK;
}

int nh_upload_bvh(nh_ctx *c, const nh_bvh_desc *b) {
    if (!c || !b) return NH_ERR_INVALID;
    if (!c->has_scene) return fail(c, "nh_upload_bvh: upload the scene first"), NH_ERR_STATE;
    HIP_TRY(c, hipSetDevice(c->device));
    if (int rc_ = pipeline_drain(c)) return rc_;
    HIP_TRY(c, hipStreamSynchronize(c->stream));
    free_all(c->bvh_bufs);
    c->has_bvh = false;
    photon_release(c);
    c->wide_w = std::getenv("NH_WIDE8") && std::getenv("NH_WIDE8")[0] == '1' ? 8 : 4;
    int top_k = nh::tree_top_nodes() * 4 / c->wide_w;
    if (const char *e = std::getenv("NH_TREE_TOP")) top_k = std::min(std::max(0, std::atoi(e)), top_k);
    nh::GpuBvh g;
    if (int rc_ = nh::build_gpu_bvh(*b, c->shapes, c->V, c->F, c->shape_bsdf_type, c->shape_bsdf_real, c->wide_w, top_k,
                                    g, c->err))
        return rc_;
    nhd::DScene &S = c->S;
    S.root_kind = g.root_kind;
    for (int i = 0; i < 3; ++i) { S.root_min[i] = g.root_min[i]; S.root_max[i] = g.root_max[i]; }
    S.iso_spheres = g.iso_spheres;
    c->tv.n_top = g.n_top;
    int rc;
    c->n_node_f4 = (int)g.nodes.size();
    c->n_leaves = (int)g.leaves.size();
    c->n_prim_f4 = (int)g.prims.size() - 3;
    drop_primary_masks(c);
    c->h_prims.clear();
    if (c->n_prim_f4 > 0 && c->n_prim_f4 / 3 <= 64)
        c->h_prims.assign(&g.prims[0].x, &g.prims[0].x + 4 * (size_t)c->n_prim_f4);
    const nh::f4 *nodes = nullptr, *prims = nullptr, *wide = nullptr;
    const nh::i2 *leaves = nullptr;
    if ((rc = upload(c, c->bvh_bufs, g.nodes.data(), g.nodes.size(), &nodes))) return rc;
    if ((rc = upload(c, c->bvh_bufs, g.leaves.data(), g.leaves.size(), &leaves))) return rc;
    if ((rc = upload(c, c->bvh_bufs, g.prims.data(), g.prims.size(), &prims))) return rc;
    if (!g.wide.empty() && (rc = upload(c, c->bvh_bufs, g.wide.data(), g.wide.size(), &wide))) return rc;
    c->tv.nodes = reinterpret_cast<const float4 *>(nodes);
    c->tv.leaves = reinterpret_cast<const int2 *>(leaves);
    c->tv.prims = reinterpret_cast<const float4 *>(prims);
    c->tv.wnodes = reinterpret_cast<const float4 *>(wide);
    c->depth_wide = g.depth_wide;
    S.nodes = c->tv.nodes;
    S.prims = c->tv.prims;
    c->bvh_indices.assign(b->indices, b->indices + b->n_indices);
    c->shape_offset = g.shape_offset;
    c->depth = (int)g.tree_depth + 2;
    if (!c->d_scene) HIP_TRY(c, hipMalloc(&c->d_scene, sizeof(nhd::DScene)));
    HIP_TRY(c, hipMemcpyAsync(c->d_scene, &c->S, sizeof(nhd::DScene), hipMemcpyHostToDevice, c->stream));
    if ((rc = build_small_image(c, g))) return rc;
    HIP_TRY(c, hipStreamSynchronize(c->stream));
    c->has_bvh = true;
    return NH_OK;
}

}
```

### optix-renderer_amd/csrc/nh_wavefront.hip

```cpp
#include "nh_dispatch.h"
#include "nh_internal.h"
#include "nh_shade.h"

#include <algorithm>
#include <cstdlib>

using namespace nhd;

#ifdef NH_DISNEY
namespace nh_disney {
#endif

namespace {

enum : int { F_DISCRETE = 1, F_NEE = 2, F_ZERO_COL = 4, F_ZNAN = 8, F_FIRST = 64 };
constexpr int kPidBits = 26;

__device__ __forceinline__ int wave_append(unsigned *counter, bool pred) {
    const unsigned long long mask = __ballot(pred);
    const int lane = threadIdx.x & 63;
    const int leader = __ffsll((long long)mask) - 1;
    unsigned base = 0;
    if (mask != 0ull && lane == leader) base = atomicAdd(counter, (unsigned)__popcll(mask));
    base = __shfl(base, leader < 0 ? 0 : leader, 64);
// ... 922 lines not shown
#pragma unroll
        for (int c = 0; c < kMatClasses; ++c) {
            const int r = wave_append(&s_n[c], cont && cls == c);
            if (cls == c) rank = r;
        }
    } else {
        cls = 0;
        rank = wave_append(&s_n[0], cont);
    }
    __syncthreads();
    if (threadIdx.x == 0) {
        unsigned tot = 0;
        for (int c = 0; c < kMatClasses; ++c) {
            s_off[c] = tot;
            tot += s_n[c];
        }
        s_base = tot ? atomicAdd(&L.cnt_out[shard * kCountStride], tot) : 0u;
    }
    __syncthreads();
    if (cont) {
        const WfBuf &Bo = L.st.buf[1 - L.in_q];
        const int slot = shard * L.seg_cap + (int)(s_base + s_off[cls]) + rank;
        store_state(Bo, slot, o);
        Bo.hit[slot] = hit_out;
    }
    if (STATS) {
        flush_trav_stats(stat_shard(L.counters), q_e, st_e);
        flush_trav_stats(stat_shard(L.counters) + kStatAny, q_s, st_s);
    }
}

__device__ __forceinline__ void store_post_head(const WfBuf &B, int s, const PathV &v, const Hit &h) {
    B.ray_o[s] = make_float4(v.org.x, v.org.y, v.org.z, 0.f);
    B.ray_d[s] = make_float4(v.d.x, v.d.y, v.d.z, __int_as_float((int)(((unsigned)(v.flags & 0x30) << kPidBits) | (unsigned)v.pid)));
    B.li[s] = make_float4(v.li.x, v.li.y, v.li.z, v.w_mats);
    B.thr[s] = make_float4(v.t.x, v.t.y, v.t.z, v.w_ems);
    B.rng[s] = v.rng.state;
    B.hit[s] = make_float4(h.t, h.u, h.v, __int_as_float(h.k));
}

struct RawState {
    float4 ro, rd, li4, th4, hv;
    uint64_t rng;
};
__device__ __forceinline__ RawState load_raw_state(const WfBuf &B, int s) {
    RawState r;
    r.ro = B.ray_o[s];
    r.rd = B.ray_d[s];
    r.li4 = B.li[s];
    r.th4 = B.thr[s];
    r.hv = B.hit[s];
    r.rng = B.rng[s];
    return r;
}

template <bool NMAP = true, class ST = DScene>
__device__ __forceinline__ void unpack_post_head(const DScene &S, const ST &T, const Traversal &tv, const WfLaunch &L,
                                                 const RawState &r, PathV &v, Hit &h, Its &its) {
    const float4 ro = r.ro, rd = r.rd, li4 = r.li4, th4 = r.th4, hv = r.hv;
    v.rng.state = r.rng;
    const int bits = __float_as_int(rd.w);
    v.flags = (int)((unsigned)bits >> kPidBits);
    v.pid = bits & ((1 << kPidBits) - 1);
    v.rng.inc = ((uint64_t)(L.s0 + v.pid / L.n_list) << 1u) | 1u;
    v.org = xyz(ro);
    v.d = xyz(rd);
    v.li = xyz(li4);
    v.w_mats = li4.w;
    v.t = xyz(th4);
    v.w_ems = th4.w;
    h.t = hv.x;
    h.u = hv.y;
    h.v = hv.z;
    h.k = __float_as_int(hv.w);
    hit_info<NMAP>(S, T.shapes, tv, h, v.org, v.d, its);
}

template <bool NMAP = true, class ST = DScene>
__device__ __forceinline__ void load_post_head(const DScene &S, const ST &T, const Traversal &tv, const WfLaunch &L,
                                               const WfBuf &B, int s, PathV &v, Hit &h, Its &its) {
    unpack_post_head<NMAP>(S, T, tv, L, load_raw_state(B, s), v, h, its);
}

template <bool ORDERED, bool STATS, bool NMAP = true, bool TRAIT = false, class ST = DScene>
__device__ __forceinline__ bool first_vertex(const DScene &S, const ST &T, const Traversal &tv, const WfLaunch &L, int s,
                                             PathV &v, Hit &h, Its &its, uint32_t *stk, int stride, TravStats &st_e,
                                             unsigned long long &q_e) {
    float4 ro, rd;
    float jx, jy;
#ifndef NH_AB_NO_PMASK
    constexpr bool MASKED = !STATS;
#else
    constexpr bool MASKED = false;
#endif
    unsigned long long cand = ~0ull;
    if constexpr (MASKED) {
        int blk;
        camera_sample<!TRAIT>(S, L, s, v.rng, ro, rd, jx, jy, &blk);
        if (L.pmask) cand = L.pmask[blk];
    } else {
        camera_sample<!TRAIT>(S, L, s, v.rng, ro, rd, jx, jy);
    }
    if (L.jit) L.jit[s] = make_float2(jx, jy);
    v.org = xyz(ro);
    v.d = xyz(rd);
    v.li = f3(0.f, 0.f, 0.f);
    v.t = f3(1.f, 1.f, 1.f);
    v.w_mats = 1.f;
    v.w_ems = 0.f;
    v.flags = F_FIRST;
    v.pid = s;
    const bool live = rd.w >= ro.w;
    q_e += live ? 1 : 0;
    const bool found =
        live && trace<16, ORDERED, false, STATS, true, 1, TRAIT, MASKED>(tv, S, v.org, v.d, ro.w, rd.w, h, stk, stride,
                                                                        st_e, cand);
    if (!shade_head<NMAP, TRAIT>(S, T, tv, v, h, found, 0.f, its)) {
        write_radiance(L, v);
        return false;
    }
    return true;
}

struct TailClocks {
    unsigned long long c[4] = {0, 0, 0, 0};
    unsigned long long bounces = 0, max_bounces = 0;
    unsigned long long cc[4] = {0, 0, 0, 0}, coop_bounces = 0;
};

template <bool ORDERED, bool STATS, bool CLK = false, int G = 1, bool FULL = true, bool NMAP = FULL, bool TRAIT = false,
          bool LEAN = false, class ST = DScene>
__device__ __forceinline__ bool rr_step(const DScene &S, const ST &T, const Traversal &tv, const WfLaunch &L, PathV &v, Its &its,
                                        Hit &h, uint32_t *stk, int stride, TravStats &st_e, TravStats &st_s,
                                        unsigned long long &q_e, unsigned long long &q_s, TailClocks *clk = nullptr) {
    const bool lead = G == 1 || (threadIdx.x & (G - 1)) == 0;
    PState o;
    bool nee = false;
    float4 so, sd;
    unsigned long long t0 = 0, t1 = 0;
    unsigned long long *cs = CLK ? (G > 1 ? clk->cc : clk->c) : nullptr;
    if constexpr (CLK) t0 = clock64();
    [[maybe_unused]] const uint64_t inc = v.rng.inc;
    shade_body<FULL, TRAIT>(S, T, tv, v, its, o, nee, so, sd);
    if constexpr (CLK) {
        t1 = clock64();
        if (lead) cs[0] += t1 - t0;
        t0 = t1;
    }
    if (nee) {
        Hit hs;
        if (lead) ++q_s;
        if (!trace<16, ORDERED, true, STATS, true, G, TRAIT>(tv, S, xyz(so), xyz(sd), so.w, sd.w, hs, stk, stride, st_s)) {
            o.li.x = o.li.x + o.pe.x;
            o.li.y = o.li.y + o.pe.y;
            o.li.z = o.li.z + o.pe.z;
            o.thr.w = o.pe.w;
        } else if (o.flags & F_ZNAN) {
            o.li.x = o.li.x + NAN;
            o.li.y = o.li.y + NAN;
            o.li.z = o.li.z + NAN;
        }
        o.flags &= ~(F_NEE | F_ZNAN);
    }
    if constexpr (CLK) {
        t1 = clock64();
        if (lead) cs[1] += t1 - t0;
        t0 = t1;
    }
    const bool live = o.rd.w >= o.ro.w;
    if (lead) q_e += live ? 1 : 0;
    const bool found = live && trace_next<16, ORDERED, STATS, true, G, FULL, TRAIT>(tv, S, h.k, xyz(o.ro), xyz(o.rd),
                                                                             o.ro.w, o.rd.w, h, stk, stride, st_e);
    if constexpr (CLK) {
        t1 = clock64();
        if (lead) cs[2] += t1 - t0;
        t0 = t1;
    }
    if constexpr (TRAIT) {
        v.org = xyz(o.ro);
        v.d = xyz(o.rd);
        v.li = xyz(o.li);
        v.w_mats = o.li.w;
        v.t = xyz(o.thr);
        v.w_ems = o.thr.w;
        v.rng.state = o.rng;
        v.rng.inc = inc;
        v.flags = o.flags;
        v.pid = o.pid;
    } else {
        v = path_of(L, o);
    }
    const bool alive = shade_head<NMAP, TRAIT, LEAN>(S, T, tv, v, h, found, o.pdfmat, its);
    if constexpr (CLK) {
        if (lead) cs[3] += clock64() - t0;
        if (lead) ++(G > 1 ? clk->coop_bounces : clk->bounces);
    }
    if (!alive) {
        if (lead) write_radiance(L, v);
        return false;
    }
    return true;
}

#ifndef NH_BOUNCE_TB
#define NH_BOUNCE_TB 256
#endif

template <bool ORDERED, bool STATS, bool FULL, bool NMAP = FULL, bool TRAIT = false, int BOUNCE = -1, class ST = DScene>
__device__ __forceinline__ bool bounce_path(const DScene &S, const ST &T, const Traversal &tv, const WfLaunch &L, const QView &qv,
                                            int q, uint32_t *my_stk, PathV &v, Hit &h, TravStats &st_e,
                                            TravStats &st_s, unsigned long long &q_e, unsigned long long &q_s,
                                            TailClocks &clk, unsigned long long &c_load, const RawState *pre = nullptr) {
    Its its;
    bool alive = true;
    unsigned long long t_ph = 0;
    if constexpr (STATS) t_ph = clock64();
    const bool first = BOUNCE < 0 ? L.first != 0 : BOUNCE == 0;
    if (first) {
        const int s = queue_slot(qv.pre, L.seg_cap, q);
        alive = first_vertex<ORDERED, STATS, NMAP, TRAIT>(S, T, tv, L, s, v, h, its, my_stk, NH_BOUNCE_TB, st_e, q_e);
    } else if (BOUNCE == 1) {
        unpack_post_head<NMAP>(S, T, tv, L, *pre, v, h, its);
    } else {
        load_post_head<NMAP>(S, T, tv, L, L.st.buf[L.in_q], queue_slot(qv.pre, L.seg_cap, q), v, h, its);
    }
    if constexpr (STATS) c_load += clock64() - t_ph;
    return alive && rr_step<ORDERED, STATS, STATS, 1, FULL, NMAP, TRAIT, true>(S, T, tv, L, v, its, h, my_stk,
                                                                         NH_BOUNCE_TB, st_e, st_s, q_e, q_s, &clk);
}

template <bool ORDERED, bool STATS, bool SORT, bool FULL = true, bool NMAP = FULL, bool TRAIT = false, int BOUNCE = -1>
__global__ __launch_bounds__(NH_BOUNCE_TB, NH_DZ_WAVES(true, NH_BOUNCE_WAVES)) void wf_bounce_rr(const DScene *__restrict__ Sp, Traversal tv_g,
                                                                     WfLaunch L) {
    __shared__ uint32_t stk[16 * NH_BOUNCE_TB];
    __shared__ unsigned s_n[kMatClasses], s_off[kMatClasses], s_base;
    extern __shared__ float4 lds_scene[];
    const QView qv = queue_view(L.cnt_in);
    const int base = blockIdx.x * NH_BOUNCE_TB;
    if (base >= qv.n) return;
    if (threadIdx.x < kMatClasses) s_n[threadIdx.x] = 0u;
    const DScene &S = *Sp;
    const int q = base + (int)threadIdx.x;
    [[maybe_unused]] RawState pre;
    if constexpr (BOUNCE == 1)
        if (q < qv.n) pre = load_raw_state(L.st.buf[L.in_q], queue_slot(qv.pre, L.seg_cap, q));
    const Traversal tv = stage_small_scene<true>(tv_g, L, lds_scene);
    const int shard = blockIdx.x & (kQueueShards - 1);
    uint32_t *my_stk = stk + threadIdx.x;
    TravStats st_e{0, 0, 0}, st_s{0, 0, 0};
    unsigned long long q_e = 0, q_s = 0;
    bool cont = false;
    PathV v;
    Hit h;
    int cls = kMatClasses - 1;
    TailClocks clk;
    unsigned long long c_load = 0, c_store = 0, t_ph = 0;
    if (q < qv.n) {
        const auto &T = scene_tables<TRAIT && NH_TRAIT_TABLES>(S, L, lds_scene);
        cont = bounce_path<ORDERED, STATS, FULL, NMAP, TRAIT, BOUNCE>(S, T, tv, L, qv, q, my_stk, v, h, st_e, st_s, q_e, q_s,
                                                                      clk, c_load, BOUNCE == 1 ? &pre : nullptr);
        if (cont) cls = prim_material(tv.prims[3 * h.k + 2]);
        if constexpr (STATS) t_ph = clock64();
    }
    int rank = 0;
    if (SORT) {
#pragma unroll
        for (int c = 0; c < kMatClasses; ++c) {
            const int r = wave_append(&s_n[c], cont && cls == c);
            if (cls == c) rank = r;
        }
    } else {
        cls = 0;
        rank = wave_append(&s_n[0], cont);
    }
    __syncthreads();
    if (threadIdx.x == 0) {
        unsigned tot = 0;
        for (int c = 0; c < kMatClasses; ++c) {
            s_off[c] = tot;
            tot += s_n[c];
        }
        s_base = tot ? atomicAdd(&L.cnt_out[shard * kCountStride], tot) : 0u;
    }
    __syncthreads();
    if (cont) store_post_head(L.st.buf[1 - L.in_q], shard * L.seg_cap + (int)(s_base + s_off[cls]) + rank, v, h);
    if (STATS) {
        if (q < qv.n) c_store = clock64() - t_ph;
        flush_trav_stats(stat_shard(L.counters), q_e, st_e);
        flush_trav_stats(stat_shard(L.counters) + kStatAny, q_s, st_s);
        unsigned long long *dst = stat_shard(L.counters) + kStatBounceClk;
        for (int j = 0; j < 7; ++j) {
            unsigned long long x = j == 0 ? c_load : j < 5 ? clk.c[j - 1] : j == 5 ? c_store : clk.bounces;
            for (int off = 32; off > 0; off >>= 1) x += __shfl_xor(x, off, 64);
            if ((threadIdx.x & 63) == 0) atomicAdd(&dst[j], x);
        }
    }
}

constexpr int kTailCoopWords = 48;
template <bool ORDERED, bool STATS, int TB, int W, bool FULL = true, bool NMAP = FULL, bool TRAIT = false>
__global__ __launch_bounds__(TB) __attribute__((amdgpu_waves_per_eu(W))) void wf_tail_rr(
    const DScene *__restrict__ Sp, Traversal tv_g, WfLaunch L, int coop) {
    __shared__ uint32_t stk[16 * TB];
    __shared__ uint32_t xfer[TB == 64 ? 4 * kTailCoopWords : 1];
    extern __shared__ float4 lds_scene[];
    const DScene &S = *Sp;
    const Traversal tv = stage_small_scene<true>(tv_g, L, lds_scene);
    const QView qv = queue_view(L.cnt_in);
    const WfBuf &B = L.st.buf[L.in_q];
    TravStats st_e{0, 0, 0}, st_s{0, 0, 0};
    unsigned long long q_e = 0, q_s = 0;
    TailClocks clk;
    const int q = blockIdx.x * TB + threadIdx.x;
    bool alive = q < qv.n;
    PathV v;
    Hit h;
    Its its;
    unsigned long long nb = 0;
    const auto &T = scene_tables<TRAIT && NH_TRAIT_TABLES>(S, L, lds_scene);
    if (alive) load_post_head<NMAP>(S, T, tv, L, B, queue_slot(qv.pre, L.seg_cap, q), v, h, its);
    const bool can_coop = TB == 64 && coop == 16;
    for (;;) {
        const unsigned long long m = __ballot(alive);
        if (m == 0ull || (can_coop && __popcll(m) <= 4)) break;
        if (alive) {
            alive = rr_step<ORDERED, STATS, STATS, 1, FULL, NMAP, TRAIT>(S, T, tv, L, v, its, h, stk + threadIdx.x, TB, st_e,
                                                                   st_s, q_e, q_s, &clk);
            ++nb;
        }
    }
    if (STATS && !can_coop) clk.max_bounces = max(clk.max_bounces, nb);
    if constexpr (TB == 64) {
        const unsigned long long m = __ballot(alive);
        if (can_coop && m) {
            const int lane = threadIdx.x & 63;
            if (alive) {
                uint32_t *w = xfer + __popcll(m & ((1ull << lane) - 1ull)) * kTailCoopWords;
                static_assert(sizeof(PathV) + sizeof(Hit) + sizeof(Its) + 8 <= kTailCoopWords * 4, "xfer slot");
                __builtin_memcpy(w, &v, sizeof(PathV));
                __builtin_memcpy(w + sizeof(PathV) / 4, &h, sizeof(Hit));
                __builtin_memcpy(w + (sizeof(PathV) + sizeof(Hit)) / 4, &its, sizeof(Its));
                __builtin_memcpy(w + (sizeof(PathV) + sizeof(Hit) + sizeof(Its)) / 4, &nb, 8);
            }
// ... 178 lines not shown
    const bool small = DEPTH == 16 && L.small_nodes + L.small_prims > 0;
    const size_t lds = small ? 16 * (size_t)(L.small_nodes + L.small_prims) + 8 * (size_t)L.small_leaves : 0;
    nh_dispatch([&](auto A, auto O, auto T, auto SM) {
        if constexpr (!SM || DEPTH == 16) {
            if constexpr (A) hipLaunchKernelGGL((wf_shadow<DEPTH, O, T, SM>), grid, dim3(128), lds, st, S, tv, L);
            else hipLaunchKernelGGL((wf_extend<DEPTH, O, T, SM>), grid, dim3(128), lds, st, S, tv, L);
        }
    }, shadow, ordered, stats, small);
}

#endif

void launch_wf_trace_deep(const DScene *S, const Traversal &tv, const WfLaunch &L, bool ordered, bool stats,
                          bool shadow, bool persistent, int wide, int bound, int depth, hipStream_t st);
#if NH_WF_HAS_PART(0) && !NH_WF_SHADING_ONLY
void launch_wf_trace(const DScene *S, const Traversal &tv, const WfLaunch &L, bool ordered, bool stats, bool shadow,
                     bool persistent, int wide, int bound, int depth, hipStream_t st) {
    if (depth <= 16) launch_wf_trace_d<16>(S, tv, L, ordered, stats, shadow, persistent, wide, bound, st);
    else if (depth <= 32) launch_wf_trace_d<32>(S, tv, L, ordered, stats, shadow, persistent, wide, bound, st);
    else launch_wf_trace_deep(S, tv, L, ordered, stats, shadow, persistent, wide, bound, depth, st);
}
#endif
#if NH_WF_HAS_PART(3) && !NH_WF_SHADING_ONLY
void launch_wf_trace_deep(const DScene *S, const Traversal &tv, const WfLaunch &L, bool ordered, bool stats,
                          bool shadow, bool persistent, int wide, int bound, int depth, hipStream_t st) {
    if (depth <= 64) launch_wf_trace_d<64>(S, tv, L, ordered, stats, shadow, persistent, wide, bound, st);
    else launch_wf_trace_d<128>(S, tv, L, ordered, stats, shadow, persistent, wide, bound, st);
}
#endif

#if NH_WF_HAS_PART(1)
#if !NH_WF_SHADING_ONLY
void launch_wf_trace2(const DScene *S, const Traversal &tv, const WfLaunch &L, bool ordered, bool stats, int wide,
                      int bound, hipStream_t st) {
    (void)ordered;
    const int want = std::max(1, (bound + 127) / 128);
    nh_dispatch([&](auto W8, auto T) {
        if constexpr (W8) launch_persistent<wf_trace_pt2<true, T, 8>>(want, st, S, tv, L);
        else launch_persistent<wf_trace_pt2<true, T>>(want, st, S, tv, L);
    }, wide == 8, stats);
}
#endif

void launch_wf_tail(const DScene *S, const Traversal &tv, const WfLaunch &L, bool ordered, bool stats, int wide,
                    int bound, int depth, hipStream_t st) {
    const dim3 grid(std::min(std::max(1, (bound + 127) / 128), wide ? kPersistentBlocks : kTraceBlocksMax));
    nh_dispatch_depth<16, 32, 64, 128>(depth, [&](auto d) {
        constexpr int DEPTH = d;
        const bool small = DEPTH == 16 && L.small_nodes + L.small_prims > 0;
        const size_t lds = small ? 16 * (size_t)(L.small_nodes + L.small_prims) + 8 * (size_t)L.small_leaves : 0;
        nh_dispatch([&](auto O, auto T, auto SM) {
            const auto launch = [&](auto kern) { hipLaunchKernelGGL(kern, grid, dim3(128), lds, st, S, tv, L); };
            if constexpr (SM) {
                if constexpr (DEPTH == 16) launch(wf_tail<DEPTH, O, T, true, 0>);
            } else if (wide == 8) {
                if constexpr (O) launch(wf_tail<DEPTH, O, T, false, 8>);
            } else if (wide) launch(wf_tail<DEPTH, O, T, false, 4>);
            else launch(wf_tail<DEPTH, O, T, false, 0>);
        }, ordered, stats, small);
    });
}

void launch_wf_bounce(const DScene *S, const Traversal &tv, const WfLaunch &L, bool ordered, bool stats, bool sort,
                      int bound, hipStream_t st) {
    int blocks = std::max(1, (bound + 255) / 256);
    blocks = (blocks + kQueueShards - 1) / kQueueShards * kQueueShards;
    const size_t lds = 16 * (size_t)rr_lds_f4(L);
    nh_dispatch([&](auto O, auto T, auto SO) {
        hipLaunchKernelGGL((wf_bounce<O, T, SO>), dim3(blocks), dim3(256), lds, st, S, tv, L);
    }, ordered, stats, sort);
}

#endif

#if NH_WF_HAS_PART(2)
void launch_wf_bounce_rr(const DScene *S, const Traversal &tv, const WfLaunch &L, bool ordered, bool stats, bool sort,
                         bool lean, bool nmap, bool trait, int bound, hipStream_t st) {
#ifndef NH_DISNEY
    if (trait && ordered && lean && !sort) return launch_wf_bounce_trait(S, tv, L, stats, bound, st);
#endif
    int blocks = std::max(1, (bound + NH_BOUNCE_TB - 1) / NH_BOUNCE_TB);
    blocks = (blocks + kQueueShards - 1) / kQueueShards * kQueueShards;
    const size_t lds = 16 * (size_t)rr_lds_f4(L);
    const auto launch = [&](auto kern) { hipLaunchKernelGGL(kern, dim3(blocks), dim3(NH_BOUNCE_TB), lds, st, S, tv, L); };
    if (ordered && lean) {
        nh_dispatch([&](auto T, auto SO) { launch(wf_bounce_rr<true, T, SO, false>); }, stats, sort);
    } else if (ordered && !nmap) {
        nh_dispatch([&](auto T, auto SO) { launch(wf_bounce_rr<true, T, SO, true, false>); }, stats, sort);
    } else {
        nh_dispatch([&](auto O, auto T, auto SO) { launch(wf_bounce_rr<O, T, SO>); }, ordered, stats, sort);
    }
}

void launch_wf_tail_rr(const DScene *S, const Traversal &tv, const WfLaunch &L, bool ordered, bool stats, int bound,
                       bool specular, bool lean, bool nmap, bool trait, hipStream_t st) {
    const char *e = std::getenv("NH_TAIL_WG");
    const int tb = e && std::atoi(e) == 256 ? 256 : 64;
    const char *w = std::getenv("NH_TAIL_RR_WAVES");
    int waves = w ? (std::atoi(w) == 1 ? 1 : std::atoi(w) == 2 ? 2 : 4) : specular ? 1 : 2;
#ifdef NH_DISNEY
    if (waves == 4) waves = 2;
#endif
    const char *ln = std::getenv("NH_TAIL_LEAN");
    if (ln && ln[0] == '0') lean = false;
    const char *cp = std::getenv("NH_TAIL_COOP");
    const int coop = cp && std::atoi(cp) == 1 ? 1 : 16;
#ifndef NH_DISNEY
    if (trait && ordered && lean && tb == 64 && waves == 2) return launch_wf_tail_trait(S, tv, L, stats, bound, coop, st);
#endif
    const dim3 grid(std::max(1, (bound + tb - 1) / tb));
    const size_t lds = 16 * (size_t)rr_lds_f4(L);
    const auto launch = [&](auto kern) { hipLaunchKernelGGL(kern, grid, dim3(tb), lds, st, S, tv, L, coop); };
    nh_dispatch([&](auto O, auto T) {
        if (tb == 256) launch(wf_tail_rr<O, T, 256, 1>);
        else if (waves == 1 && !nmap && O) launch(wf_tail_rr<O, T, 64, 1, true, false>);
        else if (waves == 1) launch(wf_tail_rr<O, T, 64, 1>);
        else if (lean && waves == 2) launch(wf_tail_rr<O, T, 64, 2, false>);
        else if (waves == 2) launch(wf_tail_rr<O, T, 64, 2>);
#ifndef NH_DISNEY
        else if (lean) launch(wf_tail_rr<O, T, 64, 4, false>);
        else launch(wf_tail_rr<O, T, 64, 4>);
#endif
    }, ordered, stats);
}

#endif

#if NH_WF_HAS_PART(4)
void launch_wf_bounce_trait(const DScene *S, const Traversal &tv, const WfLaunch &L, bool stats, int bound,
                            hipStream_t st) {
    int blocks = std::max(1, (bound + NH_BOUNCE_TB - 1) / NH_BOUNCE_TB);
    blocks = (blocks + kQueueShards - 1) / kQueueShards * kQueueShards;
    const size_t lds = 16 * (size_t)rr_lds_f4(L);
    nh_dispatch([&](auto FIRST, auto T) {
        constexpr int BOUNCE = NH_TRAIT_SPLIT ? (FIRST ? 0 : 1) : -1;
        hipLaunchKernelGGL((wf_bounce_rr<true, T, false, false, false, true, BOUNCE>), dim3(blocks), dim3(NH_BOUNCE_TB),
                           lds, st, S, tv, L);
    }, L.first != 0, stats);
}

void launch_wf_tail_trait(const DScene *S, const Traversal &tv, const WfLaunch &L, bool stats, int bound, int coop,
                          hipStream_t st) {
    const dim3 grid(std::max(1, (bound + 63) / 64));
    const size_t lds = 16 * (size_t)rr_lds_f4(L);
    nh_dispatch([&](auto T) {
        hipLaunchKernelGGL((wf_tail_rr<true, T, 64, 2, false, false, true>), grid, dim3(64), lds, st, S, tv, L, coop);
    }, stats);
}
#endif

#if NH_WF_HAS_PART(1) && !NH_WF_SHADING_ONLY
void launch_wf_camera_rays(const DScene *S, const WfLaunch &L, int bound, hipStream_t st) {
    const int blocks = std::min(std::max(1, (bound + 255) / 256), kTraceBlocksMax);
    hipLaunchKernelGGL(wf_camera_rays, dim3(blocks), dim3(256), 0, st, S, L);
}
#endif

#if NH_WF_HAS_PART(1)
#if !NH_WF_SHADING_ONLY
void launch_wf_counts(const unsigned *src, unsigned *host_dst, int n_copy, unsigned *zero, int n_zero, hipStream_t st) {
    hipLaunchKernelGGL(wf_counts_kernel, dim3(1), dim3(256), 0, st, src, host_dst, n_copy, zero, n_zero);
}

void launch_small_image(const Traversal &tv, int n_prim_f4, const int2 *slots, int pairs_off, int frames_off, float4 *image,
                        hipStream_t st) {
    hipLaunchKernelGGL(small_image_kernel, dim3(1), dim3(256), 0, st, tv.prims, n_prim_f4 / 3, slots, image + pairs_off,
                       frames_off >= 0 ? image + frames_off : nullptr);
}

void launch_wf_pack_rr(const WfLaunch &L, const WfBuf &dst, unsigned *dst_counts, int bound, hipStream_t st) {
    hipLaunchKernelGGL(wf_pack_rr, dim3(std::max(1, (bound + 255) / 256)), dim3(256), 0, st, L, dst, dst_counts);
}
#endif

void launch_wf_shade(const DScene *S, const Traversal &tv, const WfLaunch &L, bool sort, bool nmap, int bound,
                     hipStream_t st) {
    int blocks = std::max(1, (bound + 255) / 256);
    blocks = (blocks + kQueueShards - 1) / kQueueShards * kQueueShards;
    nh_dispatch([&](auto SO, auto NM) {
        hipLaunchKernelGGL((wf_shade<SO, NM>), dim3(blocks), dim3(256), 0, st, S, tv, L);
    }, sort, nmap);
}

#endif

}

#ifdef NH_DISNEY
}
#endif
```

### optix-renderer_amd/host/gpu_layout.cpp

```cpp
#include "gpu_layout.h"

#include <algorithm>
#include <cmath>
#include <cstdlib>
#include <cstring>
#include <functional>

#include "../csrc/nh_layout.h"
#include "nh_host.h"

namespace nh {

namespace {
using float4 = f4;
using int2 = i2;
struct int4 {
    int x, y, z, w;
};
inline float4 make_float4(float x, float y, float z, float w) { return float4{x, y, z, w}; }
inline int2 make_int2(int x, int y) { return int2{x, y}; }
inline int4 make_int4(int x, int y, int z, int w) { return int4{x, y, z, w}; }
inline u64x2 make_ulonglong2(uint64_t x, uint64_t y) { return u64x2{x, y}; }
}

// ... 438 lines not shown
        }
    }
    std::vector<float4> &prims = S.prims;
    prims.resize(3 * (size_t)b->n_indices);
    for (uint32_t k = 0; k < b->n_indices; ++k) {
        uint32_t g = b->indices[k];
        if (g >= off.back()) return fail("BVH index out of range"), NH_ERR_INVALID;
        uint32_t s = (uint32_t)(std::upper_bound(off.begin(), off.end(), g) - off.begin()) - 1;
        uint32_t local = g - off[s];
        const nh_shape &sh = shapes[s];
        float4 *p = &prims[3 * (size_t)k];
        int si = (int)s, one = 1, zero = 0;
        float fs, f1, f0;
        std::memcpy(&fs, &si, 4);
        std::memcpy(&f1, &one, 4);
        std::memcpy(&f0, &zero, 4);
        const int mat = shape_mat_key[s] << nhd::kPrimMatShift;
        if (sh.type == NH_SHAPE_SPHERE) {
            const int flags = 1 | mat;
            std::memcpy(&f1, &flags, 4);
            p[0] = make_float4(sh.center[0], sh.center[1], sh.center[2], sh.radius);
            p[1] = make_float4(0, 0, 0, fs);
            p[2] = make_float4(0, 0, 0, f1);
        } else {
            std::memcpy(&f0, &mat, 4);
            const uint32_t *f = &F[3 * ((size_t)sh.f_offset + local)];
            const float *p0 = &V[3 * ((size_t)sh.v_offset + f[0])], *p1 = &V[3 * ((size_t)sh.v_offset + f[1])],
                        *p2 = &V[3 * ((size_t)sh.v_offset + f[2])];
            int li = (int)local;
            float fl;
            std::memcpy(&fl, &li, 4);
            p[0] = make_float4(p0[0], p0[1], p0[2], fl);
            p[1] = make_float4(p1[0], p1[1], p1[2], fs);
            p[2] = make_float4(p2[0], p2[1], p2[2], f0);
        }
    }
    S.iso_spheres = mark_isolated_spheres(prims, nodes, leaves, S.root_kind, shape_bsdf_real);
    for (const int2 &lf : leaves)
        if (lf.y > 0) {
            float4 &w = prims[3 * ((size_t)lf.x + lf.y - 1) + 2];
            int bits;
            std::memcpy(&bits, &w.w, 4);
            bits |= nhd::kPrimLeafEnd;
            std::memcpy(&w.w, &bits, 4);
        }
    if (tree_depth + 2 > (uint32_t)nhd::kMaxStack)
        return fail("BVH deeper than " + std::to_string(nhd::kMaxStack - 2) + " levels is not supported"), NH_ERR_UNSUPPORTED;
    int depth4 = 0;
    S.wide = collapse_wide(nodes, leaves, depth4, wide_w);
    S.n_top = S.root_kind == 1 ? number_top_first(S.wide, S.root_min, S.root_max, top_k, wide_w) : 0;
    S.depth_wide = (wide_w - 1) * depth4 + 1;
    prims.resize(prims.size() + 3, make_float4(0.f, 0.f, 0.f, 0.f));
    return NH_OK;
}

PairLayout pair_layout(const i2 *leaves, int n_leaves, const f4 *prims, int n_records, bool by_kind) {
    PairLayout out;
    out.slots.assign((size_t)n_records, make_int2(-1, -1));
    out.leaves.resize((size_t)n_leaves);
    if (!by_kind) {
        for (int p = 0; p < n_records; ++p) out.slots[(size_t)p] = make_int2(p, p + 1 < n_records ? p + 1 : -1);
        for (int l = 0; l < n_leaves; ++l) out.leaves[(size_t)l] = make_int2(leaves[l].x, 0);
        return out;
    }
    std::vector<int> kind[2];
    for (int l = 0; l < n_leaves; ++l) {
        const int2 lf = leaves[l];
        kind[0].clear();
        kind[1].clear();
        for (int k = lf.x; k < lf.x + lf.y; ++k) {
            int bits;
            std::memcpy(&bits, &prims[3 * (size_t)k + 2].w, 4);
            kind[bits & nhd::kPrimSphere ? 1 : 0].push_back(k);
        }
        int p = lf.x;
        for (const std::vector<int> &v : kind)
            for (size_t i = 0; i < v.size(); i += 2) out.slots[(size_t)p++] = make_int2(v[i], i + 1 < v.size() ? v[i + 1] : -1);
        const int n_tri = ((int)kind[0].size() + 1) / 2, n_sph = ((int)kind[1].size() + 1) / 2;
        out.leaves[(size_t)l] = make_int2(lf.x, n_tri | (n_sph << 16));
    }
    return out;
}

}

extern "C" {

int nh_pair_layout(const float *records, int32_t n_records, const int32_t *leaves, int32_t n_leaves, int32_t by_kind,
                   int32_t *slots, int32_t *leaf_pairs) {
    bool ok = n_records >= 0 && n_leaves >= 0 && (n_records == 0 || (records && slots)) &&
              (n_leaves == 0 || (leaves && leaf_pairs));
    std::vector<char> used((size_t)std::max(n_records, 0), 0);
    for (int l = 0; ok && l < n_leaves; ++l) {
        const int64_t s = leaves[2 * l], n = leaves[2 * l + 1];
        ok = s >= 0 && n >= 0 && n < 65535 && s + n <= n_records;
        for (int64_t k = s; ok && k < s + n; ++k) {
            ok = !used[(size_t)k];
            used[(size_t)k] = 1;
        }
    }
    if (!ok) {
        nh::set_host_error("nh_pair_layout: invalid argument");
        return NH_ERR_INVALID;
    }
    static_assert(sizeof(nh::f4) == 4 * sizeof(float) && sizeof(nh::i2) == 2 * sizeof(int32_t), "plain arrays");
    const nh::PairLayout pl = nh::pair_layout(reinterpret_cast<const nh::i2 *>(leaves), n_leaves,
                                              reinterpret_cast<const nh::f4 *>(records), n_records, by_kind != 0);
    if (n_records > 0) std::memcpy(slots, pl.slots.data(), (size_t)n_records * sizeof(nh::i2));
    for (int l = 0; l < n_leaves; ++l) {
        leaf_pairs[3 * l] = pl.leaves[(size_t)l].x;
        leaf_pairs[3 * l + 1] = pl.leaves[(size_t)l].y & 0xffff;
        leaf_pairs[3 * l + 2] = pl.leaves[(size_t)l].y >> 16;
    }
    return NH_OK;
}

}
```

### optix-renderer_amd/host/gpu_layout.h

```cpp
#pragma once
#include <cstdint>
#include <string>
#include <vector>

#include "nori_hip.h"

namespace nh {

struct f4 {
    float x, y, z, w;
};
struct i2 {
    int x, y;
};
struct u64x2 {
    uint64_t x, y;
};

struct GpuBvh {
    std::vector<f4> nodes;
    std::vector<i2> leaves;
    std::vector<f4> prims;
    std::vector<f4> wide;
    std::vector<uint32_t> shape_offset;
    int root_kind = 0;
    float root_min[3] = {0.f, 0.f, 0.f}, root_max[3] = {0.f, 0.f, 0.f};
    uint32_t tree_depth = 0;
    int depth_wide = 1;
    int n_top = 0;
    int iso_spheres = 0;
};

int build_gpu_bvh(const nh_bvh_desc &b, const std::vector<nh_shape> &shapes, const std::vector<float> &V,
                  const std::vector<uint32_t> &F, const std::vector<int> &shape_mat_key,
                  const std::vector<int> &shape_bsdf_real, int wide_w, int top_k, GpuBvh &out, std::string &err);

std::vector<f4> collapse_wide(const std::vector<f4> &nodes, const std::vector<i2> &leaves, int &depth_out, int W = 4);
int number_top_first(std::vector<f4> &wide, const float root_min[3], const float root_max[3], int K, int W = 4);

std::vector<int> spiral_rank(int w, int h, int bs, int &nbx, int &nby);
std::vector<uint32_t> serial_ray_index(int w, int h, int bs);

struct LensTables {
    std::vector<u64x2> pix, lo;
    std::vector<uint64_t> hi;
};
LensTables lens_tables(int w, int h);

bool nee_finite(const nh_scene_desc *d);

bool primary_masks(const nh_camera &cam, const f4 *prims, int n_records, const int32_t *blocks, int n_blocks,
                   std::vector<uint64_t> &masks);
int primary_mask_pad(int width, int height);

struct PairLayout {
    std::vector<i2> slots, leaves;
};
PairLayout pair_layout(const i2 *leaves, int n_leaves, const f4 *prims, int n_records, bool by_kind);

}
```

### optix-renderer_amd/nori_hip.py

```python
from __future__ import annotations

import ctypes as C
import os

import numpy as np

_HERE = os.path.dirname(os.path.abspath(__file__))
LIB_PATH = os.environ.get("NH_LIB_PATH") or os.path.join(_HERE, "lib", "libnori_hip.so")

from nh_env import raise_hw_queues

if not os.path.exists(LIB_PATH):
    raise ImportError(f"nori_hip: HIP library not built ({LIB_PATH}); run `make` or __graft_entry__.build()")
_lib = C.CDLL(LIB_PATH)

NH_OK = 0
SHAPE_MESH, SHAPE_SPHERE = 0, 1
BSDF_DIFFUSE, BSDF_MIRROR, BSDF_DIELECTRIC, BSDF_MICROFACET = 0, 1, 2, 3
BSDF_DISNEY = 4
BSDF_QUERY_EVAL, BSDF_QUERY_SAMPLE = 0, 1
EMITTER_AREA, EMITTER_POINT, EMITTER_ENVMAP = 0, 1, 2
EMITTER_SPOT, EMITTER_DIRECTIONAL = 3, 4
EMITTER_QUERY_SAMPLE, EMITTER_QUERY_EVAL, EMITTER_QUERY_PDF = 0, 1, 2
EMITTER_QUERY_SAMPLE_STRIDE, EMITTER_QUERY_IN_STRIDE = 16, 9
# ... 82 lines not shown


def simple_denoiser(sigma_d: float = 0.0, sigma_vr: float = 0.6, range: int = 1, amount: int = 1) -> nh_denoiser:
    eps = np.float32(1e-4)

    def clampf(v, lo, hi):
        v = np.float32(v)
        return float(lo if v < lo else (hi if v > hi else v))
    d = nh_denoiser()
    d.type = DENOISER_SIMPLE
    d.sigma_d = clampf(sigma_d, eps, np.float32(10))
    d.sigma_vr = clampf(sigma_vr, eps, np.float32(10))
    d.range = int(min(max(range, 0), 50))
    d.amount = int(min(max(amount, 1), 10))
    return d


class nh_scene_desc(C.Structure):
    _fields_ = [("camera", nh_camera), ("filter", nh_filter), ("integrator", _i32), ("sample_count", _i32),
                ("n_shapes", _u32), ("shapes", C.POINTER(nh_shape)), ("n_bsdfs", _u32),
                ("bsdfs", C.POINTER(nh_bsdf)), ("n_emitters", _u32), ("emitters", C.POINTER(nh_emitter)),
                ("emitter_cdf", _fp), ("envmap", _i32), ("n_vertices", _u32), ("V", _fp), ("N", _fp),
                ("UV", _fp), ("T", _fp), ("BT", _fp), ("n_faces", _u32), ("F", _u32p), ("n_area_cdf", _u32),
                ("area_cdf", _fp), ("env", nh_envmap), ("denoiser", nh_denoiser), ("n_textures", _u32),
                ("textures", C.POINTER(nh_texture)), ("n_texels", C.c_uint64), ("texels", _fp),
                ("normals_direction", _f * 3), ("emitter_ext", C.POINTER(nh_emitter_ext)),
                ("n_media", _u32), ("media", C.POINTER(nh_medium)), ("shape_medium", _u32p),
                ("ambient_medium", _u32), ("sampler", _i32), ("adaptive_initial_uniform", _i32)]


class nh_bvh_node(C.Structure):
    _fields_ = [("word0", _u32), ("word1", _u32), ("bbox_min", _f * 3), ("bbox_max", _f * 3)]


class nh_bvh_desc(C.Structure):
    _fields_ = [("n_nodes", _u32), ("nodes", C.POINTER(nh_bvh_node)), ("n_indices", _u32), ("indices", _u32p),
                ("n_shapes", _u32), ("shape_offset", _u32p), ("bbox_min", _f * 3), ("bbox_max", _f * 3),
                ("max_depth", _u32)]


class nh_ray_soa(C.Structure):
    _fields_ = [(n, _fp) for n in ("ox", "oy", "oz", "dx", "dy", "dz", "mint", "maxt")]


class nh_hit_soa(C.Structure):
    _fields_ = [("hit", C.POINTER(C.c_uint8)), ("t", _fp), ("u", _fp), ("v", _fp), ("prim", _u32p),
                ("shape", _u32p)]


class nh_render_req(C.Structure):
    _fields_ = [("sample_begin", _i32), ("sample_end", _i32), ("seed", C.c_uint64), ("n_blocks", _i32),
                ("blocks", C.POINTER(_i32)), ("mode", _i32), ("traversal", _i32), ("clear", _i32),
                ("collect_stats", _i32)]


class nh_adaptive_stats(C.Structure):
    _fields_ = [("total_samples", C.c_uint64), ("passes", C.c_uint64), ("max_passes", C.c_uint64),
                ("n_blocks", C.c_uint64)]


class nh_render_stats(C.Structure):
    _fields_ = [("kernel_ms_path", C.c_double), ("kernel_ms_splat", C.c_double), ("kernel_ms_extend", C.c_double),
                ("kernel_ms_shadow", C.c_double), ("kernel_ms_shade", C.c_double), ("launches_path", C.c_uint64),
                ("launches_splat", C.c_uint64), ("launches_extend", C.c_uint64), ("launches_shadow", C.c_uint64),
                ("launches_shade", C.c_uint64), ("samples", C.c_uint64), ("ray_queries", C.c_uint64),
                ("nodes_visited", C.c_uint64), ("boxes_tested", C.c_uint64), ("prims_tested", C.c_uint64),
                ("invalid_samples", C.c_uint64), ("shadow_queries", C.c_uint64),
                ("shadow_nodes_visited", C.c_uint64), ("shadow_boxes_tested", C.c_uint64),
                ("shadow_prims_tested", C.c_uint64), ("shade_state_bytes", C.c_uint64),
                ("extend_queue_bytes", C.c_uint64), ("shadow_queue_bytes", C.c_uint64),
                ("paths_shaded", C.c_uint64), ("kernel_ms_tail", C.c_double), ("launches_tail", C.c_uint64),
                ("node_bytes", C.c_uint64)] + [
        (n, C.c_uint64) for n in ("tail_queries", "tail_nodes_visited", "tail_boxes_tested", "tail_prims_tested",
                                  "tail_shadow_queries", "tail_shadow_nodes_visited", "tail_shadow_boxes_tested",
                                  "tail_shadow_prims_tested", "lds_scene", "fused_bounce", "comm_inits")] + [
        ("kernel_ms_denoise", C.c_double), ("launches_denoise", C.c_uint64), ("tails_async", C.c_uint64),
        ("pools_active", C.c_uint64), ("trace_fused", C.c_uint64)] + [
        (n, C.c_uint64) for n in ("tail_cycles_body", "tail_cycles_shadow", "tail_cycles_closest", "tail_cycles_head",
                                  "tail_bounces", "tail_max_bounces", "tail_coop_cycles_body",
                                  "tail_coop_cycles_shadow", "tail_coop_cycles_closest", "tail_coop_cycles_head",
                                  "tail_coop_bounces", "bounce_cycles_load", "bounce_cycles_body",
                                  "bounce_cycles_shadow", "bounce_cycles_closest", "bounce_cycles_head",
                                  "bounce_cycles_store", "bounce_bounces", "bounce_traits", "primary_masks",
                                  "pair_kinds")]


def _sig(name, res, *args):
    fn = getattr(_lib, name)
    fn.restype = res
    fn.argtypes = list(args)
    return fn


_vp = C.c_void_p
_sig("nh_scene_load_xml", _i32, C.c_char_p, C.POINTER(_vp))
_sig("nh_scene_load_xml_index", _i32, C.c_char_p, _i32, C.POINTER(_vp))
_sig("nh_scene_get_desc", _i32, _vp, C.POINTER(nh_scene_desc))
_sig("nh_scene_set_resolution", _i32, _vp, _i32, _i32)
_sig("nh_scene_set_sample_count", _i32, _vp, _i32)
_sig("nh_scene_set_sampler", _i32, _vp, _i32, _i32)
_sig("nh_scene_set_bsdf", _i32, _vp, _u32, C.POINTER(nh_bsdf))
_sig("nh_scene_set_integrator", _i32, _vp, _i32)
_sig("nh_scene_add_texture", _u32, _vp, C.POINTER(nh_texture), _fp)
_sig("nh_scene_set_normal_map", _i32, _vp, _u32, _u32)
_sig("nh_scene_set_lens_draw_order", _i32, _vp, _i32)
_sig("nh_texture_decode", _i32, C.POINTER(C.c_uint8), C.c_uint64, _i32, _fp)
_sig("nh_scene_free", None, _vp)
_sig("nh_host_last_error", C.c_char_p)
_sig("nh_debug_transform", _i32, C.c_char_p, _fp, _i32)
_sig("nh_bvh_build", _i32, C.POINTER(nh_scene_desc), _i32, C.POINTER(_vp))
_sig("nh_bvh_get_desc", _i32, _vp, C.POINTER(nh_bvh_desc))
_sig("nh_bvh_free", None, _vp)
_sig("nh_primary_masks", _i32, C.POINTER(nh_camera), _fp, _i32, C.POINTER(_i32), _i32, C.POINTER(C.c_uint64),
     C.POINTER(_i32))
_sig("nh_primary_mask_pad", _i32, _i32, _i32)
_sig("nh_pair_layout", _i32, _fp, _i32, C.POINTER(_i32), _i32, _i32, C.POINTER(_i32), C.POINTER(_i32))
_sig("nh_framebuffer_to_rgb", _i32, _fp, _i32, _i32, _i32, _fp)
_sig("nh_write_pfm", _i32, C.c_char_p, _fp, _i32, _i32)
_sig("nh_image_load_png", _i32, C.c_char_p, C.POINTER(C.c_uint8), C.c_size_t, C.POINTER(_i32), C.POINTER(_i32))
_sig("nh_write_exr", _i32, C.c_char_p, _fp, _i32, _i32)
_sig("nh_write_png", _i32, C.c_char_p, _fp, _i32, _i32)
_sig("nh_rgb_to_ldr", _i32, _fp, _i32, _i32, C.POINTER(C.c_uint8))
_sig("nh_get_device_count", _i32, C.POINTER(C.c_int))
_sig("nh_create", _i32, C.c_int, C.POINTER(_vp))
_sig("nh_destroy", None, _vp)
_sig("nh_upload_scene", _i32, _vp, C.POINTER(nh_scene_desc))
_sig("nh_upload_bvh", _i32, _vp, C.POINTER(nh_bvh_desc))
_sig("nh_trace_rays", _i32, _vp, C.POINTER(nh_ray_soa), _i32, _i32, _i32, C.POINTER(nh_hit_soa))
_sig("nh_render", _i32, _vp, C.POINTER(nh_render_req))
_sig("nh_synchronize", _i32, _vp)
_sig("nh_get_framebuffer", _i32, _vp, _fp, C.c_size_t)
_sig("nh_framebuffer_device_ptr", _i32, _vp, C.POINTER(_vp), C.POINTER(C.c_size_t))
_sig("nh_get_stats", _i32, _vp, C.POINTER(nh_render_stats))
_sig("nh_reset_stats", _i32, _vp)
_sig("nh_get_adaptive_stats", _i32, _vp, C.POINTER(nh_adaptive_stats))
_sig("nh_get_adaptive_variance", _i32, _vp, _fp, C.c_size_t)
_sig("nh_reduce_framebuffers", _i32, C.POINTER(_vp), _i32, _i32)
_sig("nh_denoise", _i32, _vp, C.POINTER(nh_denoiser))
_sig("nh_denoise_image", _i32, _vp, _fp, _i32, _i32, _i32, C.POINTER(nh_denoiser))
_sig("nh_bsdf_query", _i32, _vp, C.POINTER(nh_bsdf), _fp, _i32, _i32, _fp, _fp, _fp, _fp, _fp, _fp, C.POINTER(_i32))
_sig("nh_emitter_query", _i32, _vp, _u32, _i32, _i32, _fp, _fp, _fp)
_sig("nh_medium_query", _i32, _vp, _u32, _i32, _i32, _fp, _fp)
_sig("nh_last_error", C.c_char_p, _vp)


class nh_test_desc(C.Structure):
    _fields_ = [("type", _i32), ("significance_level", _f), ("sample_count", _i32), ("n_angles", _u32),
                ("angles", _fp), ("n_references", _u32), ("references", _fp), ("n_scenes", _u32), ("n_bsdfs", _u32),
                ("bsdfs", C.POINTER(nh_bsdf))]


class nh_test_result(C.Structure):
    _fields_ = [("mean", C.c_double), ("variance", C.c_double), ("reference", C.c_double), ("p_value", C.c_double),
                ("accepted", _i32), ("sample_count", _i32), ("angle", _f), ("pad", _i32)]


TEST_TTEST, TEST_CHI2TEST = 0, 1
RADIANCE_QUERY_MAX = 1 << 24
_dp = C.POINTER(C.c_double)
_i32p = C.POINTER(_i32)
_sig("nh_test_load_xml", _i32, C.c_char_p, C.POINTER(_vp))
_sig("nh_test_get_desc", _i32, _vp, C.POINTER(nh_test_desc))
_sig("nh_test_free", None, _vp)
_sig("nh_students_t_test", _i32, C.c_double, C.c_double, C.c_double, _i32, C.c_double, _i32, _i32p, _dp)
_sig("nh_radiance_query", _i32, _vp, C.c_uint64, _i32, _i32p, _i32p, _fp, _fp, _fp)
_sig("nh_ttest_scene", _i32, _vp, C.c_uint64, C.c_int64, _i32, _dp, _dp, _fp)
_sig("nh_ttest_bsdf", _i32, _vp, C.POINTER(nh_bsdf), _fp, _f, C.c_uint64, _i32, _dp, _dp, _fp)
_sig("nh_test_run", _i32, C.c_int, C.c_char_p, C.c_uint64, C.POINTER(nh_test_result), _i32, _i32p)


INTEGRATOR_PHOTONMAPPER = 9
EMITTER_QUERY_SAMPLE_PHOTON, EMITTER_QUERY_PHOTON_STRIDE = 3, 12
PHOTON_QUERY_CODEC, PHOTON_QUERY_GATHER = 0, 1
PHOTON_STREAM = 1 << 32
PHOTON_DEFAULT_BATCH = 1 << 18


class nh_photon_params(C.Structure):
    _fields_ = [("photon_count", _i32), ("photon_radius", _f)]


class nh_photon_stats(C.Structure):
    _fields_ = [("stored", _i32), ("emitted", _i32), ("radius", _f), ("cell_size", _f),
                ("occupied_cells", C.c_uint64)]


_u8p = C.POINTER(C.c_uint8)
_sig("nh_scene_get_photon_params", _i32, _vp, C.POINTER(nh_photon_params))
_sig("nh_scene_set_photon_params", _i32, _vp, C.POINTER(nh_photon_params))
_sig("nh_photon_tables", _i32, _fp, _fp, _fp, _fp, _fp)
_sig("nh_photon_map_build", _i32, _vp, C.POINTER(nh_photon_params), C.c_uint64, _i32)
_sig("nh_get_photon_stats", _i32, _vp, C.POINTER(nh_photon_stats))
_sig("nh_get_photons", _i32, _vp, _i32, _i32, _fp, _fp, _fp, _u8p, _i32p, _i32p)
_sig("nh_photon_query", _i32, _vp, _i32, _i32, _fp, _u8p, _i32p, _fp)


INTEGRATOR_AV, INTEGRATOR_ENVMAPTESTER = 10, 11


# ... 465 lines not shown
        if mode in (None, EMITTER_QUERY_PDF):
            out["pdf"] = call(EMITTER_QUERY_PDF, inp, np.zeros(m, np.float32))
        return out

    def medium_query(self, medium: int, mode: int, inp: np.ndarray) -> np.ndarray:
        n_in, n_out = {MEDIUM_QUERY_FREE_PATH: (2, 2), MEDIUM_QUERY_TRANSMITTANCE: (6, 3),
                       MEDIUM_QUERY_PHASE_SAMPLE: (2, 4), MEDIUM_QUERY_PHASE_PDF: (3, 1)}[mode]
        inp = np.ascontiguousarray(inp, dtype=np.float32).reshape(-1, n_in)
        out = np.zeros((len(inp), n_out), np.float32)
        self._check(_lib.nh_medium_query(self._h, medium, mode, len(inp), _fptr(inp), _fptr(out)), "medium_query")
        return out[:, 0] if n_out == 1 else out

    def radiance_query(self, pixel, sample, seed: int = 0, pixel_sample=None) -> dict:
        pixel = np.ascontiguousarray(pixel, dtype=np.int32).ravel()
        sample = np.ascontiguousarray(np.broadcast_to(np.asarray(sample, dtype=np.int32), pixel.shape))
        n = len(pixel)
        ps = None if pixel_sample is None else np.ascontiguousarray(pixel_sample, dtype=np.float32).reshape(n, 2)
        out = {"rgb": np.zeros((n, 3), np.float32), "jitter": np.zeros((n, 2), np.float32)}
        self._check(_lib.nh_radiance_query(self._h, seed, n, pixel.ctypes.data_as(_i32p), sample.ctypes.data_as(_i32p),
                                           None if ps is None else _fptr(ps), _fptr(out["rgb"]), _fptr(out["jitter"])),
                    "radiance_query")
        return out

    def ttest_scene(self, n: int, seed: int = 0, first: int = 0, luminance: bool = False):
        m, v = C.c_double(0.0), C.c_double(0.0)
        lum = np.zeros(max(n, 0), np.float32) if luminance else None
        self._check(_lib.nh_ttest_scene(self._h, seed, first, n, C.byref(m), C.byref(v),
                                        None if lum is None else _fptr(lum)), "ttest_scene")
        return (m.value, v.value, lum) if luminance else (m.value, v.value)

    def ttest_bsdf(self, bsdf: nh_bsdf, angle_deg: float, n: int, first_draw: int = 0, albedo=None,
                   luminance: bool = False):
        m, v = C.c_double(0.0), C.c_double(0.0)
        lum = np.zeros(max(n, 0), np.float32) if luminance else None
        alb = None if albedo is None else np.ascontiguousarray(albedo, dtype=np.float32).reshape(3)
        self._check(_lib.nh_ttest_bsdf(self._h, C.byref(bsdf), None if alb is None else _fptr(alb), angle_deg, first_draw,
                                       n, C.byref(m), C.byref(v), None if lum is None else _fptr(lum)), "ttest_bsdf")
        return (m.value, v.value, lum) if luminance else (m.value, v.value)

    def trace(self, o: np.ndarray, d: np.ndarray, mint: np.ndarray, maxt: np.ndarray, any_hit=False,
              traversal: int = TRAVERSAL_REFERENCE) -> dict:
        n = len(o)
        cols = [np.ascontiguousarray(x, dtype=np.float32) for x in (o[:, 0], o[:, 1], o[:, 2], d[:, 0], d[:, 1],
                                                                     d[:, 2], mint, maxt)]
        r = nh_ray_soa(*[_fptr(c) for c in cols])
        res = {"hit": np.zeros(n, np.uint8), "t": np.zeros(n, np.float32), "u": np.zeros(n, np.float32),
               "v": np.zeros(n, np.float32), "prim": np.zeros(n, np.uint32), "shape": np.zeros(n, np.uint32)}
        h = nh_hit_soa(res["hit"].ctypes.data_as(C.POINTER(C.c_uint8)), _fptr(res["t"]), _fptr(res["u"]),
                       _fptr(res["v"]), res["prim"].ctypes.data_as(_u32p), res["shape"].ctypes.data_as(_u32p))
        self._check(_lib.nh_trace_rays(self._h, C.byref(r), n, int(any_hit), traversal, C.byref(h)), "trace_rays")
        return res


def tile_shard(width: int, height: int, world: int, rank: int) -> list:
    nbx, nby = (width + 31) // 32, (height + 31) // 32
    return [b for b in range(nbx * nby) if b % world == rank]


def primary_mask_pad(width: int, height: int) -> int:
    return int(_lib.nh_primary_mask_pad(width, height))


def primary_masks(camera: nh_camera, records: np.ndarray, blocks):
    rec = np.ascontiguousarray(records, dtype=np.float32).reshape(-1, 12)
    blk = np.ascontiguousarray(blocks, dtype=np.int32).ravel()
    out = np.zeros(len(blk), np.uint64)
    built = _i32(0)
    _host_check(_lib.nh_primary_masks(C.byref(camera), _fptr(rec), len(rec), blk.ctypes.data_as(C.POINTER(_i32)),
                                      len(blk), out.ctypes.data_as(C.POINTER(C.c_uint64)), C.byref(built)),
                "primary_masks")
    return out if built.value else None


def pair_layout(records: np.ndarray, leaves, by_kind: bool = True):
    rec = np.ascontiguousarray(records, dtype=np.float32).reshape(-1, 12)
    lv = np.ascontiguousarray(leaves, dtype=np.int32).reshape(-1, 2)
    slots, lp = np.zeros((len(rec), 2), np.int32), np.zeros((len(lv), 3), np.int32)
    ip = C.POINTER(_i32)
    _host_check(_lib.nh_pair_layout(_fptr(rec), len(rec), lv.ctypes.data_as(ip), len(lv), 1 if by_kind else 0,
                                    slots.ctypes.data_as(ip), lp.ctypes.data_as(ip)), "pair_layout")
    return slots, lp


def reduce_framebuffers(ctxs, root: int = 0):
    arr = (_vp * len(ctxs))(*[c._h for c in ctxs])
    rc = _lib.nh_reduce_framebuffers(arr, len(ctxs), root)
    if rc != NH_OK:
        raise NoriError(f"nh_reduce_framebuffers failed ({rc})")


def to_rgb(rgbw: np.ndarray, border: int) -> np.ndarray:
    h, w = rgbw.shape[0] - 2 * border, rgbw.shape[1] - 2 * border
    src = np.ascontiguousarray(rgbw, dtype=np.float32)
    out = np.zeros((h, w, 3), np.float32)
    rc = _lib.nh_framebuffer_to_rgb(_fptr(src), w, h, border, _fptr(out))
    if rc != NH_OK:
        raise NoriError("framebuffer_to_rgb failed")
    return out


def write_exr(path: str, rgb: np.ndarray):
    rgb = np.ascontiguousarray(rgb, dtype=np.float32)
    _host_check(_lib.nh_write_exr(path.encode(), _fptr(rgb), rgb.shape[1], rgb.shape[0]), "write_exr")


def write_png(path: str, rgb: np.ndarray):
    rgb = np.ascontiguousarray(rgb, dtype=np.float32)
    _host_check(_lib.nh_write_png(path.encode(), _fptr(rgb), rgb.shape[1], rgb.shape[0]), "write_png")


def rgb_to_ldr(rgb: np.ndarray) -> np.ndarray:
    rgb = np.ascontiguousarray(rgb, dtype=np.float32)
    out = np.empty(rgb.shape[:2] + (3,), np.uint8)
    _host_check(_lib.nh_rgb_to_ldr(_fptr(rgb), rgb.shape[1], rgb.shape[0],
                                   out.ctypes.data_as(C.POINTER(C.c_uint8))), "rgb_to_ldr")
    return out


def write_pfm(path: str, rgb: np.ndarray):
    rgb = np.ascontiguousarray(rgb, dtype=np.float32)
    _host_check(_lib.nh_write_pfm(path.encode(), _fptr(rgb), rgb.shape[1], rgb.shape[0]), "write_pfm")


def load_png(path: str) -> np.ndarray:
    w, h = _i32(), _i32()
    _host_check(_lib.nh_image_load_png(path.encode(), None, 0, C.byref(w), C.byref(h)), "load_png")
    out = np.zeros((h.value, w.value, 4), np.uint8)
    _host_check(_lib.nh_image_load_png(path.encode(), out.ctypes.data_as(C.POINTER(C.c_uint8)), out.nbytes,
                                       C.byref(w), C.byref(h)), "load_png")
    return out
```

Before: 7750 Msamples/s.

## Add flat stackless traversal for one- or two-leaf BVH scenes

For tiny scenes whose BVH is a single leaf or a root with two leaves (at most 16 primitive pairs), the host builds a flat image: root and leaf boxes in a header, followed by the packed triangle and sphere pairs. The wavefront bounce and first-vertex kernels get a FLAT template path that tests these boxes directly and walks both leaves without a stack or node fetches, for both closest-hit and shadow rays. This is meant to remove stack traffic and node-loop overhead on the Cornell box. It adds another kernel instantiation, and the result must match ordered traversal tie-breaking, which flat_combine reproduces.

```diff
diff --git a/include/nori_hip.h b/include/nori_hip.h
--- a/include/nori_hip.h
+++ b/include/nori_hip.h
@@ -277,6 +277,7 @@
     uint64_t bounce_traits;
     uint64_t primary_masks;
     uint64_t pair_kinds;
+    uint64_t flat_trace;
 } nh_render_stats;
 
 typedef struct nh_scene nh_scene;
@@ -321,6 +322,9 @@
 
 int nh_pair_layout(const float *records, int32_t n_records, const int32_t *leaves, int32_t n_leaves, int32_t by_kind,
                    int32_t *slots, int32_t *leaf_pairs);
+
+int nh_flat_image(const float *records, int32_t n_records, const int32_t *leaves, int32_t n_leaves, const float *boxes,
+                  int32_t allowed, float *image, int32_t image_cap_f4, int32_t *n_f4, int32_t *box_equal);
 
 int nh_framebuffer_to_rgb(const float *rgbw, int32_t width, int32_t height, int32_t border, float *rgb);
 int nh_write_pfm(const char *path, const float *rgb, int32_t width, int32_t height);
diff --git a/optix-renderer_amd/csrc/nh_ctx.h b/optix-renderer_amd/csrc/nh_ctx.h
--- a/optix-renderer_amd/csrc/nh_ctx.h
+++ b/optix-renderer_amd/csrc/nh_ctx.h
@@ -172,6 +172,7 @@
     int small_tab[5] = {0, 0, 0, 0, 0};
     bool pair_kinds = false;
     float4 *small_image_ref = nullptr;
+    const float4 *flat_image = nullptr;
     nh_camera camera{};
     std::vector<float> h_prims;
     unsigned long long *pmask = nullptr;
diff --git a/optix-renderer_amd/csrc/nh_flat_combine.h b/optix-renderer_amd/csrc/nh_flat_combine.h
--- /dev/null
+++ b/optix-renderer_amd/csrc/nh_flat_combine.h
@@ -0,0 +1,38 @@
+#pragma once
+
+#if defined(__HIPCC__) || defined(__CUDACC__)
+#define NH_FLAT_HD __host__ __device__ __forceinline__
+#else
+#define NH_FLAT_HD inline
+#endif
+
+namespace nhd {
+
+struct FlatBest {
+    float t, u, v;
+    int k;
+    bool found;
+};
+
+template <bool ORDERED>
+NH_FLAT_HD bool flat_combine(bool hl, bool hr, float nl, float nr, float maxt, const FlatBest &L, const FlatBest &R,
+                             FlatBest &out) {
+    const bool both = hl && hr;
+    const bool right_first = both ? (ORDERED && nr < nl) : hr;
+    const FlatBest &F = right_first ? R : L, &S = right_first ? L : R;
+    const bool found_first = (hl || hr) && F.found;
+    const float maxt1 = found_first ? F.t : maxt;
+    const int k_first = found_first ? F.k : -1;
+    const float near_second = right_first ? nl : nr;
+    const bool take_second = both && near_second <= maxt1 && S.found && S.t <= maxt1 && (S.t < maxt1 || S.k > k_first);
+    out.t = take_second ? S.t : F.t;
+    out.u = take_second ? S.u : F.u;
+    out.v = take_second ? S.v : F.v;
+    out.k = take_second ? S.k : k_first;
+    out.found = found_first || take_second;
+    return out.found;
+}
+
+NH_FLAT_HD bool flat_combine_any(bool hl, bool hr, bool any_l, bool any_r) { return (hl && any_l) || (hr && any_r); }
+
+}
diff --git a/optix-renderer_amd/csrc/nh_internal.h b/optix-renderer_amd/csrc/nh_internal.h
--- a/optix-renderer_amd/csrc/nh_internal.h
+++ b/optix-renderer_amd/csrc/nh_internal.h
@@ -173,6 +173,7 @@
     unsigned long long *counters;
     const unsigned long long *pmask;
     int pmask_nbx;
+    const float4 *flat;
 };
 constexpr int kPersistentBlocks = 256 * 16;
 constexpr size_t kSmallSceneBytes = 16384;
diff --git a/optix-renderer_amd/csrc/nh_layout.h b/optix-renderer_amd/csrc/nh_layout.h
--- a/optix-renderer_amd/csrc/nh_layout.h
+++ b/optix-renderer_amd/csrc/nh_layout.h
@@ -10,6 +10,10 @@
 constexpr int kWideF4 = 8;
 constexpr int kWideEmpty = (int)0x80000000;
 
+constexpr int kPairF4 = 6;
+constexpr int kFlatHeaderF4 = 6, kFlatMaxPairs = 16;
+constexpr int kFlatLeftEq = 1, kFlatRightEq = 2;
+
 constexpr int kMaxStack = 128;
 
 }
diff --git a/optix-renderer_amd/csrc/nh_pipeline.hip b/optix-renderer_amd/csrc/nh_pipeline.hip
--- a/optix-renderer_amd/csrc/nh_pipeline.hip
+++ b/optix-renderer_amd/csrc/nh_pipeline.hip
@@ -218,6 +218,9 @@
     L.pmask_nbx = c->nbx;
     c->stats.primary_masks = masks ? 1 : 0;
     c->stats.pair_kinds = p.fused && c->pair_kinds && !j.stats ? 1 : 0;
+    const bool flat = p.rr && c->flat_image && c->pair_kinds && !j.stats && !c->disney;
+    L.flat = flat ? c->flat_image : nullptr;
+    c->stats.flat_trace = flat ? 1 : 0;
     c->stats.fused_bounce = p.fused ? 1 : 0;
     c->stats.node_bytes = p.wide ? 16 * nhd::kWideF4 * (c->wide_w / 4) : 64;
     c->stats.lds_scene = small && !p.persistent && c->depth <= 16 ? 1 : 0;
@@ -817,6 +820,7 @@
     if (av_split && av_wide(c, q)) c->stats.node_bytes = 16 * nhd::kWideF4 * (c->wide_w / 4);
     c->stats.primary_masks = 0;
     c->stats.pair_kinds = 0;
+    c->stats.flat_trace = 0;
     c->stats.trace_fused = 0;
     c->stats.lds_scene = 0;
     c->stats.fused_bounce = 0;
diff --git a/optix-renderer_amd/csrc/nh_traverse.h b/optix-renderer_amd/csrc/nh_traverse.h
--- a/optix-renderer_amd/csrc/nh_traverse.h
+++ b/optix-renderer_amd/csrc/nh_traverse.h
@@ -1,5 +1,6 @@
 #pragma once
 #include "nh_device.h"
+#include "nh_flat_combine.h"
 
 namespace nhd {
 
@@ -215,7 +216,6 @@
     const float4 *frames;
     int n_top;
 };
-constexpr int kPairF4 = 6;
 
 NHD bool prim_is_tri(float4 c) { return (__float_as_int(c.w) & kPrimSphere) == 0; }
 NHD int prim_material(float4 c) { return (__float_as_int(c.w) >> kPrimMatShift) & 3; }
@@ -523,6 +523,101 @@
     return ANY ? false : found;
 }
 
+template <bool ANY, bool MASKED>
+NHD bool flat_leaf(const float4 *__restrict__ pp, int n_tri, int n_sph, F3 o, F3 d, float mint, float maxt, Hit &best,
+                   bool &found, unsigned long long cand) {
+    bool any = false;
+    for (int i = 0; i < n_tri; ++i, pp += kPairF4) {
+        const float4 q5 = pp[5];
+        const int k0 = __float_as_int(q5.z), k1 = __float_as_int(q5.w);
+        if constexpr (MASKED)
+            if (!(((cand >> (k0 & 63)) | (cand >> (k1 & 63))) & 1ull)) continue;
+        const float4 q0 = pp[0], q1 = pp[1], q2 = pp[2], q3 = pp[3], q4 = pp[4];
+        const P3 p0{f2{q0.x, q0.y}, f2{q0.z, q0.w}, f2{q1.x, q1.y}};
+        const P3 e1{f2{q2.x, q2.y}, f2{q2.z, q2.w}, f2{q3.x, q3.y}};
+        const P3 e2{f2{q3.z, q3.w}, f2{q4.x, q4.y}, f2{q4.z, q4.w}};
+        f2 pt, pu, pv;
+        bool ok0, ok1;
+        tri_test_pair_e(p0, e1, e2, o, d, mint, pt, pu, pv, ok0, ok1);
+        if (ANY) {
+            any = any || (ok0 && pt.x <= maxt) || (ok1 && pt.y <= maxt);
+            continue;
+        }
+        accept_hit(ok0 && pt.x <= maxt, pt.x, pu.x, pv.x, k0, maxt, best, found);
+        accept_hit(ok1 && pt.y <= maxt, pt.y, pu.y, pv.y, k1, maxt, best, found);
+    }
+    for (int i = 0; i < n_sph; ++i, pp += kPairF4) {
+        const float4 q5 = pp[5];
+        const int k0 = __float_as_int(q5.z), k1 = __float_as_int(q5.w);
+        if constexpr (MASKED)
+            if (!(((cand >> (k0 & 63)) | (cand >> (k1 & 63))) & 1ull)) continue;
+        const float4 q0 = pp[0], q1 = pp[1];
+        f2 tmin, tmax;
+        bool ok0, ok1;
+        sphere_test_pair(f2{q0.x, q0.y}, f2{q0.z, q0.w}, f2{q1.x, q1.y}, f2{q1.z, q1.w}, o, d, tmin, tmax, ok0, ok1);
+        if (!(ok0 | ok1)) continue;
+        float t0, t1;
+        const bool h0 = sphere_in_range(tmin.x, tmax.x, mint, maxt, t0) && ok0;
+        if (ANY) {
+            any = any || h0 || (sphere_in_range(tmin.y, tmax.y, mint, maxt, t1) && ok1);
+            continue;
+        }
+        accept_hit(h0, t0, 0.f, 0.f, k0, maxt, best, found);
+        const bool h1 = sphere_in_range(tmin.y, tmax.y, mint, maxt, t1) && ok1;
+        accept_hit(h1, t1, 0.f, 0.f, k1, maxt, best, found);
+    }
+    return any;
+}
+
+template <bool ORDERED, bool ANY, bool RCP, bool MASKED = false>
+NHD bool trace_flat(const float4 *__restrict__ fl, const DScene &S, F3 o, F3 d, float mint, float maxt, Hit &best,
+                    unsigned long long cand = ~0ull) {
+    if (mint == kEps) mint = e_max(mint, mint * e_max(fabsf(o.x), e_max(fabsf(o.y), fabsf(o.z))));
+    best.k = -1;
+    best.t = INFINITY;
+    if (S.root_kind == 0 || maxt < mint) return false;
+    const F3 r = RCP ? f3(dir_rcp(d.x), dir_rcp(d.y), dir_rcp(d.z)) : f3(1.0f / d.x, 1.0f / d.y, 1.0f / d.z);
+    const bool fin = isfinite(r.x) & isfinite(r.y) & isfinite(r.z);
+    const float4 h0 = fl[0], h1 = fl[1], h2 = fl[2], h3 = fl[3], h4 = fl[4], h5 = fl[5];
+    const auto box = [&](float4 mn, float4 mx, float &near_t) {
+        return fin ? box_test_finite(mn.x, mn.y, mn.z, mx.x, mx.y, mx.z, o, r, mint, maxt, near_t)
+                   : box_test(mn.x, mn.y, mn.z, mx.x, mx.y, mx.z, o, d, r, mint, maxt, near_t);
+    };
+    float near_root;
+    if (!box(h0, h1, near_root)) return false;
+    const int eq = __float_as_int(h0.w);
+    const bool two = __float_as_int(h1.w) == 2;
+    bool hl = true, hr = false;
+    float nl = near_root, nr = near_root;
+    if (!(eq & kFlatLeftEq)) hl = box(h2, h3, nl);
+    if (two) {
+        hr = true;
+        if (!(eq & kFlatRightEq)) hr = box(h4, h5, nr);
+    }
+    const int cl = __float_as_int(h2.w), cr = __float_as_int(h4.w);
+    const float4 *pl = fl + kFlatHeaderF4, *pr = pl + kPairF4 * ((cl & 0xffff) + (cl >> 16));
+    Hit bl{INFINITY, 0.f, 0.f, -1}, br{INFINITY, 0.f, 0.f, -1};
+    bool fl_found = false, fr_found = false, any_l = false, any_r = false;
+    if (hl) any_l = flat_leaf<ANY, MASKED>(pl, cl & 0xffff, cl >> 16, o, d, mint, maxt, bl, fl_found, cand);
+    if constexpr (ANY) {
+        if (hr && !any_l) any_r = flat_leaf<ANY, MASKED>(pr, cr & 0xffff, cr >> 16, o, d, mint, maxt, br, fr_found, cand);
+        return flat_combine_any(hl, hr, any_l, any_r);
+    } else {
+        const bool left_first = hl && !(hr && ORDERED && nr < nl);
+        const float maxt_l = fl_found ? bl.t : maxt;
+        if (hr && !(left_first && !(nr <= maxt_l)))
+            flat_leaf<ANY, MASKED>(pr, cr & 0xffff, cr >> 16, o, d, mint, maxt, br, fr_found, cand);
+        FlatBest out;
+        flat_combine<ORDERED>(hl, hr, nl, nr, maxt, FlatBest{bl.t, bl.u, bl.v, bl.k, fl_found},
+                              FlatBest{br.t, br.u, br.v, br.k, fr_found}, out);
+        best.t = out.found ? out.t : INFINITY;
+        best.u = out.u;
+        best.v = out.v;
+        best.k = out.k;
+        return out.found;
+    }
+}
+
 template <bool STATS, int G = 1>
 NHD bool iso_sphere_hit(const Traversal &tv, int k_prev, F3 o, F3 d, float mint, float maxt, Hit &best,
                         TravStats &st) {
@@ -552,6 +647,16 @@
         return true;
 #endif
     return trace<DEPTH, ORDERED, false, STATS, PAIRS, G, RCP>(tv, S, o, d, mint, maxt, best, stk, stride, st);
+}
+template <bool ORDERED, bool ISO = true, bool RCP = false>
+NHD bool trace_next_flat(const float4 *__restrict__ fl, const Traversal &tv, const DScene &S, int k_prev, F3 o, F3 d,
+                         float mint, float maxt, Hit &best) {
+#ifndef NH_AB_NO_ISO
+    TravStats none{0, 0, 0};
+    if (ISO && S.iso_spheres && S.root_kind != 0 && iso_sphere_hit<false, 1>(tv, k_prev, o, d, mint, maxt, best, none))
+        return true;
+#endif
+    return trace_flat<ORDERED, false, RCP>(fl, S, o, d, mint, maxt, best);
 }
 
 
diff --git a/optix-renderer_amd/csrc/nh_upload.hip b/optix-renderer_amd/csrc/nh_upload.hip
--- a/optix-renderer_amd/csrc/nh_upload.hip
+++ b/optix-renderer_amd/csrc/nh_upload.hip
@@ -386,6 +386,7 @@
     c->h_area_cdf.assign(d->area_cdf, d->area_cdf + d->n_area_cdf);
     c->n_emit_faces = (int)ef_tri.size();
     c->small_image = c->small_image_ref = nullptr;
+    c->flat_image = nullptr;
     c->pair_kinds = false;
     c->V.assign(d->V, d->V + 3 * nv);
     c->F.assign(d->F, d->F + 3 * (size_t)d->n_faces);
@@ -419,6 +420,7 @@
 
 static int build_small_image(nh_ctx *c, const nh::GpuBvh &g) {
     c->small_image = c->small_image_ref = nullptr;
+    c->flat_image = nullptr;
     c->pair_kinds = false;
     for (int &v : c->small_tab) v = 0;
     const size_t scene_bytes = 16 * (size_t)(c->n_node_f4 + c->n_prim_f4) + 8 * (size_t)c->n_leaves;
@@ -497,6 +499,36 @@
         }
         HIP_TRY(c, hipStreamSynchronize(c->stream));
         (pass == 0 ? c->small_image : c->small_image_ref) = img;
+    }
+    const bool one_leaf = g.root_kind == 2 && c->n_leaves == 1;
+    bool two_leaves = g.root_kind == 1 && c->n_node_f4 == 4 && c->n_leaves == 2;
+    if (two_leaves) {
+        int refs[2];
+        std::memcpy(refs, &g.nodes[3].x, sizeof(refs));
+        two_leaves = refs[0] == ~0 && refs[1] == ~1;
+    }
+    if (c->pair_kinds && (one_leaf || two_leaves)) {
+        float boxes[18];
+        for (int i = 0; i < 3; ++i) {
+            boxes[i] = g.root_min[i];
+            boxes[3 + i] = g.root_max[i];
+        }
+        if (two_leaves) {
+            const nh::f4 n0 = g.nodes[0], n1 = g.nodes[1], n2 = g.nodes[2];
+            const float lr[12] = {n0.x, n0.y, n0.z, n0.w, n1.x, n1.y, n1.z, n1.w, n2.x, n2.y, n2.z, n2.w};
+            std::memcpy(boxes + 6, lr, sizeof(lr));
+        } else {
+            std::memcpy(boxes + 6, boxes, 6 * sizeof(float));
+            std::memcpy(boxes + 12, boxes, 6 * sizeof(float));
+        }
+        const nh::PairLayout pl = nh::pair_layout(g.leaves.data(), c->n_leaves, g.prims.data(), n, true);
+        const nh::FlatImage fi = nh::flat_image(boxes, g.leaves.data(), c->n_leaves, g.prims.data(), n, pl, nh::flat_trace_knob());
+        if (fi.flat) {
+            const nh::f4 *dev = nullptr;
+            if (int rc = upload(c, c->bvh_bufs, fi.data.data(), fi.data.size(), &dev)) return rc;
+            HIP_TRY(c, hipStreamSynchronize(c->stream));
+            c->flat_image = reinterpret_cast<const float4 *>(dev);
+        }
     }
     return NH_OK;
 }
diff --git a/optix-renderer_amd/csrc/nh_wavefront.hip b/optix-renderer_amd/csrc/nh_wavefront.hip
--- a/optix-renderer_amd/csrc/nh_wavefront.hip
+++ b/optix-renderer_amd/csrc/nh_wavefront.hip
@@ -1028,10 +1028,10 @@
     unpack_post_head<NMAP>(S, T, tv, L, load_raw_state(B, s), v, h, its);
 }
 
-template <bool ORDERED, bool STATS, bool NMAP = true, bool TRAIT = false, class ST = DScene>
+template <bool ORDERED, bool STATS, bool NMAP = true, bool TRAIT = false, bool FLAT = false, class ST = DScene>
 __device__ __forceinline__ bool first_vertex(const DScene &S, const ST &T, const Traversal &tv, const WfLaunch &L, int s,
                                              PathV &v, Hit &h, Its &its, uint32_t *stk, int stride, TravStats &st_e,
-                                             unsigned long long &q_e) {
+                                             unsigned long long &q_e, const float4 *__restrict__ flat = nullptr) {
     float4 ro, rd;
     float jx, jy;
 #ifndef NH_AB_NO_PMASK
@@ -1058,9 +1058,12 @@
     v.pid = s;
     const bool live = rd.w >= ro.w;
     q_e += live ? 1 : 0;
-    const bool found =
-        live && trace<16, ORDERED, false, STATS, true, 1, TRAIT, MASKED>(tv, S, v.org, v.d, ro.w, rd.w, h, stk, stride,
-                                                                        st_e, cand);
+    bool found;
+    if constexpr (FLAT)
+        found = live && trace_flat<ORDERED, false, TRAIT, MASKED>(flat, S, v.org, v.d, ro.w, rd.w, h, cand);
+    else
+        found = live && trace<16, ORDERED, false, STATS, true, 1, TRAIT, MASKED>(tv, S, v.org, v.d, ro.w, rd.w, h, stk,
+                                                                                stride, st_e, cand);
     if (!shade_head<NMAP, TRAIT>(S, T, tv, v, h, found, 0.f, its)) {
         write_radiance(L, v);
         return false;
@@ -1075,10 +1078,12 @@
 };
 
 template <bool ORDERED, bool STATS, bool CLK = false, int G = 1, bool FULL = true, bool NMAP = FULL, bool TRAIT = false,
-          bool LEAN = false, class ST = DScene>
+          bool LEAN = false, bool FLAT = false, class ST = DScene>
 __device__ __forceinline__ bool rr_step(const DScene &S, const ST &T, const Traversal &tv, const WfLaunch &L, PathV &v, Its &its,
                                         Hit &h, uint32_t *stk, int stride, TravStats &st_e, TravStats &st_s,
-                                        unsigned long long &q_e, unsigned long long &q_s, TailClocks *clk = nullptr) {
+                                        unsigned long long &q_e, unsigned long long &q_s, TailClocks *clk = nullptr,
+                                        const float4 *__restrict__ flat = nullptr) {
+    static_assert(!FLAT || (G == 1 && !STATS), "the flat traversal carries one ray per lane and counts nothing");
     const bool lead = G == 1 || (threadIdx.x & (G - 1)) == 0;
     PState o;
     bool nee = false;
@@ -1096,7 +1101,10 @@
     if (nee) {
         Hit hs;
         if (lead) ++q_s;
-        if (!trace<16, ORDERED, true, STATS, true, G, TRAIT>(tv, S, xyz(so), xyz(sd), so.w, sd.w, hs, stk, stride, st_s)) {
+        bool occluded;
+        if constexpr (FLAT) occluded = trace_flat<ORDERED, true, TRAIT>(flat, S, xyz(so), xyz(sd), so.w, sd.w, hs);
+        else occluded = trace<16, ORDERED, true, STATS, true, G, TRAIT>(tv, S, xyz(so), xyz(sd), so.w, sd.w, hs, stk, stride, st_s);
+        if (!occluded) {
             o.li.x = o.li.x + o.pe.x;
             o.li.y = o.li.y + o.pe.y;
             o.li.z = o.li.z + o.pe.z;
@@ -1115,8 +1123,12 @@
     }
     const bool live = o.rd.w >= o.ro.w;
     if (lead) q_e += live ? 1 : 0;
-    const bool found = live && trace_next<16, ORDERED, STATS, true, G, FULL, TRAIT>(tv, S, h.k, xyz(o.ro), xyz(o.rd),
-                                                                             o.ro.w, o.rd.w, h, stk, stride, st_e);
+    bool found;
+    if constexpr (FLAT)
+        found = live && trace_next_flat<ORDERED, FULL, TRAIT>(flat, tv, S, h.k, xyz(o.ro), xyz(o.rd), o.ro.w, o.rd.w, h);
+    else
+        found = live && trace_next<16, ORDERED, STATS, true, G, FULL, TRAIT>(tv, S, h.k, xyz(o.ro), xyz(o.rd), o.ro.w,
+                                                                            o.rd.w, h, stk, stride, st_e);
     if constexpr (CLK) {
         t1 = clock64();
         if (lead) cs[2] += t1 - t0;
@@ -1152,11 +1164,13 @@
 #define NH_BOUNCE_TB 256
 #endif
 
-template <bool ORDERED, bool STATS, bool FULL, bool NMAP = FULL, bool TRAIT = false, int BOUNCE = -1, class ST = DScene>
+template <bool ORDERED, bool STATS, bool FULL, bool NMAP = FULL, bool TRAIT = false, int BOUNCE = -1, bool FLAT = false,
+          class ST = DScene>
 __device__ __forceinline__ bool bounce_path(const DScene &S, const ST &T, const Traversal &tv, const WfLaunch &L, const QView &qv,
                                             int q, uint32_t *my_stk, PathV &v, Hit &h, TravStats &st_e,
                                             TravStats &st_s, unsigned long long &q_e, unsigned long long &q_s,
-                                            TailClocks &clk, unsigned long long &c_load, const RawState *pre = nullptr) {
+                                            TailClocks &clk, unsigned long long &c_load, const RawState *pre = nullptr,
+                                            const float4 *__restrict__ flat = nullptr) {
     Its its;
     bool alive = true;
     unsigned long long t_ph = 0;
@@ -1164,21 +1178,24 @@
     const bool first = BOUNCE < 0 ? L.first != 0 : BOUNCE == 0;
     if (first) {
         const int s = queue_slot(qv.pre, L.seg_cap, q);
-        alive = first_vertex<ORDERED, STATS, NMAP, TRAIT>(S, T, tv, L, s, v, h, its, my_stk, NH_BOUNCE_TB, st_e, q_e);
+        alive = first_vertex<ORDERED, STATS, NMAP, TRAIT, FLAT>(S, T, tv, L, s, v, h, its, my_stk, NH_BOUNCE_TB, st_e, q_e,
+                                                                flat);
     } else if (BOUNCE == 1) {
         unpack_post_head<NMAP>(S, T, tv, L, *pre, v, h, its);
     } else {
         load_post_head<NMAP>(S, T, tv, L, L.st.buf[L.in_q], queue_slot(qv.pre, L.seg_cap, q), v, h, its);
     }
     if constexpr (STATS) c_load += clock64() - t_ph;
-    return alive && rr_step<ORDERED, STATS, STATS, 1, FULL, NMAP, TRAIT, true>(S, T, tv, L, v, its, h, my_stk,
-                                                                         NH_BOUNCE_TB, st_e, st_s, q_e, q_s, &clk);
-}
-
-template <bool ORDERED, bool STATS, bool SORT, bool FULL = true, bool NMAP = FULL, bool TRAIT = false, int BOUNCE = -1>
+    return alive && rr_step<ORDERED, STATS, STATS, 1, FULL, NMAP, TRAIT, true, FLAT>(S, T, tv, L, v, its, h, my_stk, NH_BOUNCE_TB,
+                                                                               st_e, st_s, q_e, q_s, &clk, flat);
+}
+
+template <bool ORDERED, bool STATS, bool SORT, bool FULL = true, bool NMAP = FULL, bool TRAIT = false, int BOUNCE = -1,
+          bool FLAT = false>
 __global__ __launch_bounds__(NH_BOUNCE_TB, NH_DZ_WAVES(true, NH_BOUNCE_WAVES)) void wf_bounce_rr(const DScene *__restrict__ Sp, Traversal tv_g,
-                                                                     WfLaunch L) {
-    __shared__ uint32_t stk[16 * NH_BOUNCE_TB];
+                                                                     WfLaunch L, const float4 *__restrict__ flat) {
+    static_assert(!(FLAT && STATS), "the counting kernels walk the tree");
+    __shared__ uint32_t stk[FLAT ? 1 : 16 * NH_BOUNCE_TB];
     __shared__ unsigned s_n[kMatClasses], s_off[kMatClasses], s_base;
     extern __shared__ float4 lds_scene[];
     const QView qv = queue_view(L.cnt_in);
@@ -1192,7 +1209,7 @@
         if (q < qv.n) pre = load_raw_state(L.st.buf[L.in_q], queue_slot(qv.pre, L.seg_cap, q));
     const Traversal tv = stage_small_scene<true>(tv_g, L, lds_scene);
     const int shard = blockIdx.x & (kQueueShards - 1);
-    uint32_t *my_stk = stk + threadIdx.x;
+    uint32_t *my_stk = FLAT ? stk : stk + threadIdx.x;
     TravStats st_e{0, 0, 0}, st_s{0, 0, 0};
     unsigned long long q_e = 0, q_s = 0;
     bool cont = false;
@@ -1203,8 +1220,8 @@
     unsigned long long c_load = 0, c_store = 0, t_ph = 0;
     if (q < qv.n) {
         const auto &T = scene_tables<TRAIT && NH_TRAIT_TABLES>(S, L, lds_scene);
-        cont = bounce_path<ORDERED, STATS, FULL, NMAP, TRAIT, BOUNCE>(S, T, tv, L, qv, q, my_stk, v, h, st_e, st_s, q_e, q_s,
-                                                                      clk, c_load, BOUNCE == 1 ? &pre : nullptr);
+        cont = bounce_path<ORDERED, STATS, FULL, NMAP, TRAIT, BOUNCE, FLAT>(S, T, tv, L, qv, q, my_stk, v, h, st_e, st_s, q_e,
+                                                                            q_s, clk, c_load, BOUNCE == 1 ? &pre : nullptr, flat);
         if (cont) cls = prim_material(tv.prims[3 * h.k + 2]);
         if constexpr (STATS) t_ph = clock64();
     }
@@ -1549,13 +1566,26 @@
     int blocks = std::max(1, (bound + NH_BOUNCE_TB - 1) / NH_BOUNCE_TB);
     blocks = (blocks + kQueueShards - 1) / kQueueShards * kQueueShards;
     const size_t lds = 16 * (size_t)rr_lds_f4(L);
-    const auto launch = [&](auto kern) { hipLaunchKernelGGL(kern, dim3(blocks), dim3(NH_BOUNCE_TB), lds, st, S, tv, L); };
+    const auto launch = [&](auto kern) {
+        hipLaunchKernelGGL(kern, dim3(blocks), dim3(NH_BOUNCE_TB), lds, st, S, tv, L, L.flat);
+    };
+#ifndef NH_DISNEY
+    const bool flat = L.flat != nullptr && !stats;
+#else
+    const bool flat = false;
+#endif
     if (ordered && lean) {
-        nh_dispatch([&](auto T, auto SO) { launch(wf_bounce_rr<true, T, SO, false>); }, stats, sort);
+        nh_dispatch([&](auto T, auto SO, auto FL) {
+            if constexpr (!(T && FL) && !(kDisney && FL)) launch(wf_bounce_rr<true, T, SO, false, false, false, -1, FL>);
+        }, stats, sort, flat);
     } else if (ordered && !nmap) {
-        nh_dispatch([&](auto T, auto SO) { launch(wf_bounce_rr<true, T, SO, true, false>); }, stats, sort);
+        nh_dispatch([&](auto T, auto SO, auto FL) {
+            if constexpr (!(T && FL) && !(kDisney && FL)) launch(wf_bounce_rr<true, T, SO, true, false, false, -1, FL>);
+        }, stats, sort, flat);
     } else {
-        nh_dispatch([&](auto O, auto T, auto SO) { launch(wf_bounce_rr<O, T, SO>); }, ordered, stats, sort);
+        nh_dispatch([&](auto O, auto T, auto SO, auto FL) {
+            if constexpr (!(T && FL) && !(kDisney && FL)) launch(wf_bounce_rr<O, T, SO, true, true, false, -1, FL>);
+        }, ordered, stats, sort, flat);
     }
 }
 
@@ -1599,11 +1629,12 @@
     int blocks = std::max(1, (bound + NH_BOUNCE_TB - 1) / NH_BOUNCE_TB);
     blocks = (blocks + kQueueShards - 1) / kQueueShards * kQueueShards;
     const size_t lds = 16 * (size_t)rr_lds_f4(L);
-    nh_dispatch([&](auto FIRST, auto T) {
+    nh_dispatch([&](auto FIRST, auto T, auto FL) {
         constexpr int BOUNCE = NH_TRAIT_SPLIT ? (FIRST ? 0 : 1) : -1;
-        hipLaunchKernelGGL((wf_bounce_rr<true, T, false, false, false, true, BOUNCE>), dim3(blocks), dim3(NH_BOUNCE_TB),
-                           lds, st, S, tv, L);
-    }, L.first != 0, stats);
+        if constexpr (!(T && FL))
+            hipLaunchKernelGGL((wf_bounce_rr<true, T, false, false, false, true, BOUNCE, FL>), dim3(blocks),
+                               dim3(NH_BOUNCE_TB), lds, st, S, tv, L, L.flat);
+    }, L.first != 0, stats, L.flat != nullptr && !stats);
 }
 
 void launch_wf_tail_trait(const DScene *S, const Traversal &tv, const WfLaunch &L, bool stats, int bound, int coop,
diff --git a/optix-renderer_amd/host/gpu_layout.cpp b/optix-renderer_amd/host/gpu_layout.cpp
--- a/optix-renderer_amd/host/gpu_layout.cpp
+++ b/optix-renderer_amd/host/gpu_layout.cpp
@@ -544,9 +544,94 @@
     return out;
 }
 
+bool flat_trace_knob() {
+    const char *e = std::getenv("NH_FLAT_TRACE");
+    return !(e && e[0] == '0');
+}
+
+FlatImage flat_image(const float boxes[18], const i2 *leaves, int n_leaves, const f4 *prims, int n_records,
+                     const PairLayout &pl, bool allowed) {
+    FlatImage out;
+    if (!allowed || n_leaves < 1 || n_leaves > 2 || n_records < 1 || (int)pl.leaves.size() != n_leaves) return out;
+    int n_pairs = 0;
+    for (int l = 0; l < n_leaves; ++l) {
+        const int2 p = pl.leaves[(size_t)l];
+        if (p.y == 0 && leaves[l].y > 0) return out;
+        n_pairs += (p.y & 0xffff) + (p.y >> 16);
+    }
+    if (n_pairs < 1 || n_pairs > nhd::kFlatMaxPairs) return out;
+    const auto same_bits = [](const float *a, const float *b) { return std::memcmp(a, b, 6 * sizeof(float)) == 0; };
+    const auto as_float = [](int v) {
+        float f;
+        std::memcpy(&f, &v, 4);
+        return f;
+    };
+    const float *root = boxes, *lb = n_leaves == 2 ? boxes + 6 : boxes, *rb = n_leaves == 2 ? boxes + 12 : boxes;
+    out.box_equal = n_leaves == 1 ? nhd::kFlatLeftEq
+                                  : (same_bits(lb, root) ? nhd::kFlatLeftEq : 0) | (same_bits(rb, root) ? nhd::kFlatRightEq : 0);
+    out.data.reserve((size_t)nhd::kFlatHeaderF4 + (size_t)nhd::kPairF4 * n_pairs);
+    out.data.push_back(make_float4(root[0], root[1], root[2], as_float(out.box_equal)));
+    out.data.push_back(make_float4(root[3], root[4], root[5], as_float(n_leaves)));
+    out.data.push_back(make_float4(lb[0], lb[1], lb[2], as_float(pl.leaves[0].y)));
+    out.data.push_back(make_float4(lb[3], lb[4], lb[5], 0.f));
+    out.data.push_back(make_float4(rb[0], rb[1], rb[2], as_float(n_leaves == 2 ? pl.leaves[1].y : 0)));
+    out.data.push_back(make_float4(rb[3], rb[4], rb[5], 0.f));
+    for (int l = 0; l < n_leaves; ++l) {
+        const int2 p = pl.leaves[(size_t)l];
+        for (int i = 0, n = (p.y & 0xffff) + (p.y >> 16); i < n; ++i) {
+            const int2 s = pl.slots[(size_t)(p.x + i)];
+            const int k = s.x, k1 = s.y < 0 ? k : s.y;
+            if (k < 0 || k >= n_records || k1 >= n_records) return FlatImage{};
+            const float4 a = prims[3 * (size_t)k], b = prims[3 * (size_t)k + 1], c = prims[3 * (size_t)k + 2];
+            const float4 a1 = prims[3 * (size_t)k1], b1 = prims[3 * (size_t)k1 + 1], c1 = prims[3 * (size_t)k1 + 2];
+            out.data.push_back(make_float4(a.x, a1.x, a.y, a1.y));
+            out.data.push_back(make_float4(a.z, a1.z, a.w, a1.w));
+            out.data.push_back(make_float4(b.x - a.x, b1.x - a1.x, b.y - a.y, b1.y - a1.y));
+            out.data.push_back(make_float4(b.z - a.z, b1.z - a1.z, c.x - a.x, c1.x - a1.x));
+            out.data.push_back(make_float4(c.y - a.y, c1.y - a1.y, c.z - a.z, c1.z - a1.z));
+            out.data.push_back(make_float4(c.w, c1.w, as_float(k), as_float(k1)));
+        }
+    }
+    out.flat = true;
+    return out;
+}
+
 }
 
 extern "C" {
+
+int nh_flat_image(const float *records, int32_t n_records, const int32_t *leaves, int32_t n_leaves, const float *boxes,
+                  int32_t allowed, float *image, int32_t image_cap_f4, int32_t *n_f4, int32_t *box_equal) {
+    bool ok = n_records >= 0 && n_leaves >= 0 && (n_records == 0 || records) && (n_leaves == 0 || leaves) && boxes &&
+              n_f4 && box_equal && image_cap_f4 >= 0 && (image_cap_f4 == 0 || image);
+    std::vector<char> used((size_t)std::max(n_records, 0), 0);
+    for (int l = 0; ok && l < n_leaves; ++l) {
+        const int64_t s = leaves[2 * l], n = leaves[2 * l + 1];
+        ok = s >= 0 && n >= 0 && n < 65535 && s + n <= n_records;
+        for (int64_t k = s; ok && k < s + n; ++k) {
+            ok = !used[(size_t)k];
+            used[(size_t)k] = 1;
+        }
+    }
+    if (!ok) {
+        nh::set_host_error("nh_flat_image: invalid argument");
+        return NH_ERR_INVALID;
+    }
+    const nh::i2 *lv = reinterpret_cast<const nh::i2 *>(leaves);
+    const nh::f4 *rec = reinterpret_cast<const nh::f4 *>(records);
+    const nh::PairLayout pl = nh::pair_layout(lv, n_leaves, rec, n_records, true);
+    const nh::FlatImage fi = nh::flat_image(boxes, lv, n_leaves, rec, n_records, pl, allowed != 0 && nh::flat_trace_knob());
+    *n_f4 = fi.flat ? (int32_t)fi.data.size() : 0;
+    *box_equal = fi.box_equal;
+    if (fi.flat) {
+        if ((size_t)image_cap_f4 < fi.data.size()) {
+            nh::set_host_error("nh_flat_image: image buffer too small");
+            return NH_ERR_INVALID;
+        }
+        std::memcpy(image, fi.data.data(), fi.data.size() * sizeof(nh::f4));
+    }
+    return NH_OK;
+}
 
 int nh_pair_layout(const float *records, int32_t n_records, const int32_t *leaves, int32_t n_leaves, int32_t by_kind,
                    int32_t *slots, int32_t *leaf_pairs) {
diff --git a/optix-renderer_amd/host/gpu_layout.h b/optix-renderer_amd/host/gpu_layout.h
--- a/optix-renderer_amd/host/gpu_layout.h
+++ b/optix-renderer_amd/host/gpu_layout.h
@@ -58,4 +58,13 @@
 };
 PairLayout pair_layout(const i2 *leaves, int n_leaves, const f4 *prims, int n_records, bool by_kind);
 
+struct FlatImage {
+    bool flat = false;
+    int box_equal = 0;
+    std::vector<f4> data;
+};
+FlatImage flat_image(const float boxes[18], const i2 *leaves, int n_leaves, const f4 *prims, int n_records,
+                     const PairLayout &pl, bool allowed);
+bool flat_trace_knob();
+
 }
diff --git a/optix-renderer_amd/nori_hip.py b/optix-renderer_amd/nori_hip.py
--- a/optix-renderer_amd/nori_hip.py
+++ b/optix-renderer_amd/nori_hip.py
@@ -188,7 +188,7 @@
                                   "tail_coop_bounces", "bounce_cycles_load", "bounce_cycles_body",
                                   "bounce_cycles_shadow", "bounce_cycles_closest", "bounce_cycles_head",
                                   "bounce_cycles_store", "bounce_bounces", "bounce_traits", "primary_masks",
-                                  "pair_kinds")]
+                                  "pair_kinds", "flat_trace")]
 
 
 def _sig(name, res, *args):
@@ -221,6 +221,7 @@
      C.POINTER(_i32))
 _sig("nh_primary_mask_pad", _i32, _i32, _i32)
 _sig("nh_pair_layout", _i32, _fp, _i32, C.POINTER(_i32), _i32, _i32, C.POINTER(_i32), C.POINTER(_i32))
+_sig("nh_flat_image", _i32, _fp, _i32, C.POINTER(_i32), _i32, _fp, _i32, _fp, _i32, C.POINTER(_i32), C.POINTER(_i32))
 _sig("nh_framebuffer_to_rgb", _i32, _fp, _i32, _i32, _i32, _fp)
 _sig("nh_write_pfm", _i32, C.c_char_p, _fp, _i32, _i32)
 _sig("nh_image_load_png", _i32, C.c_char_p, C.POINTER(C.c_uint8), C.c_size_t, C.POINTER(_i32), C.POINTER(_i32))
@@ -852,6 +853,18 @@
     return slots, lp
 
 
+def flat_image(records: np.ndarray, leaves, boxes, allowed: bool = True):
+    rec = np.ascontiguousarray(records, dtype=np.float32).reshape(-1, 12)
+    lv = np.ascontiguousarray(leaves, dtype=np.int32).reshape(-1, 2)
+    bx = np.ascontiguousarray(boxes, dtype=np.float32).ravel()
+    assert bx.size == 18
+    cap = 6 + 6 * 16
+    img, n, eq = np.zeros((cap, 4), np.float32), _i32(0), _i32(0)
+    _host_check(_lib.nh_flat_image(_fptr(rec), len(rec), lv.ctypes.data_as(C.POINTER(_i32)), len(lv), _fptr(bx),
+                                   1 if allowed else 0, _fptr(img), cap, C.byref(n), C.byref(eq)), "flat_image")
+    return (img[:n.value].copy() if n.value else None), int(eq.value)
+
+
 def reduce_framebuffers(ctxs, root: int = 0):
     arr = (_vp * len(ctxs))(*[c._h for c in ctxs])
     rc = _lib.nh_reduce_framebuffers(arr, len(ctxs), root)
```

Measured after the change: 8771 Msamples/s, median of 6. 1.13x the previous value.
